# rushi-the-neural-arch/PyTorch-DistributedTraining

Measured on AMD Instinct MI355X. Metric: tokens/sec GPT-2-1.3B FSDP (whole node), higher is better.
Workload: dtype bf16; 1 GPU; model=gpt2-1.3b, global_batch=96, seq_len=1024, parallelism=fsdp1, micro_batch_per_gpu=96, params=1313722368, hip_graph=False, optimizer=fused AdamW + global-norm clip

## Files before the change

### csrc/kernels/gelu.h

```cpp
#pragma once
#include <hip/hip_runtime.h>

namespace pdt {

constexpr float kSqrt2OverPi = 0.7978845608028654f;
constexpr float kGeluC = 0.044715f;
constexpr float kInvSqrt2 = 0.7071067811865476f;

constexpr float kGeluA = -2.f * 0.7978845608028654f * 1.4426950408889634f;
constexpr float kGeluB = kGeluA * 0.044715f;
__device__ __forceinline__ float sigmoid2z(float u) {
  const float a = u * __builtin_fmaf(kGeluB, u * u, kGeluA);
  return __builtin_amdgcn_rcpf(1.f + __builtin_amdgcn_exp2f(a));
}

typedef float gelu_f32x2 __attribute__((ext_vector_type(2)));
constexpr float kGeluD1 = 2.f * 0.7978845608028654f;
constexpr float kGeluD3 = kGeluD1 * 3.f * 0.044715f;
__device__ __forceinline__ void gelu_fwd_grad2(gelu_f32x2 u, gelu_f32x2& y, gelu_f32x2& d) {
  const gelu_f32x2 u2 = u * u;
  const gelu_f32x2 a = u * __builtin_elementwise_fma(gelu_f32x2{kGeluB, kGeluB}, u2, gelu_f32x2{kGeluA, kGeluA});
  const gelu_f32x2 e = gelu_f32x2{__builtin_amdgcn_exp2f(a[0]), __builtin_amdgcn_exp2f(a[1])} + gelu_f32x2{1.f, 1.f};
  const gelu_f32x2 s = gelu_f32x2{__builtin_amdgcn_rcpf(e[0]), __builtin_amdgcn_rcpf(e[1])};
  y = u * s;
  const gelu_f32x2 t = __builtin_elementwise_fma(-s, s, s);
  const gelu_f32x2 q = __builtin_elementwise_fma(gelu_f32x2{kGeluD3, kGeluD3}, u2, gelu_f32x2{kGeluD1, kGeluD1});
  d = __builtin_elementwise_fma(u * t, q, s);
}

template <bool TANH>
__device__ __forceinline__ float gelu_f(float u) {
  if (TANH) {
    return u * sigmoid2z(u);
  } else {
    return 0.5f * u * (1.f + erff(u * kInvSqrt2));
  }
}
template <bool TANH>
__device__ __forceinline__ float gelu_grad(float u) {
  if (TANH) {
    const float s = sigmoid2z(u);
    return s + 2.f * u * s * (1.f - s) * kSqrt2OverPi * (1.f + 3.f * kGeluC * u * u);
  } else {
    const float cdf = 0.5f * (1.f + erff(u * kInvSqrt2));
    const float pdf = 0.3989422804014327f * __expf(-0.5f * u * u);
    return cdf + u * pdf;
  }
}

}
```

### csrc/kernels/gemm.hip

```cpp
#include "common.h"
#include "gelu.h"
#include "reduce.h"
#include <stdlib.h>
#include <type_traits>

using namespace pdt;

namespace {

typedef __bf16 bf16x8_t __attribute__((ext_vector_type(8)));
typedef short v4i16 __attribute__((ext_vector_type(4)));
typedef int v4i __attribute__((ext_vector_type(4)));
typedef __attribute__((address_space(3))) v4i16 lds_v4i16;
typedef __attribute__((address_space(3))) u16x8 lds_u16x8;
typedef __attribute__((address_space(3))) void lds_void;
typedef __attribute__((address_space(3))) const char lds_cchar;

constexpr int TM = 256, TN = 256, KB = 64, NTH = 256;
constexpr int OPB = TM * KB * 2;
constexpr int STB = 2 * OPB;
constexpr int PIECES = OPB / (NTH * 16);

enum { L_NT = 0, L_TT = 1 };
enum { E_PLAIN = 0, E_BIAS = 1, E_GELU = 2, E_DGELU = 3, E_F32 = 4 };

__device__ __forceinline__ f32x4 mfma16(const u16x8& a, const u16x8& b, const f32x4& c) {
  return __builtin_amdgcn_mfma_f32_16x16x32_bf16(__builtin_bit_cast(bf16x8_t, a), __builtin_bit_cast(bf16x8_t, b),
                                                 c, 0, 0, 0);
}

__device__ __forceinline__ int tt_f(int r) { return 2 * ((r & 3) | ((r >> 1) & 4)); }

template <int LAYOUT>
struct Dma {
  uint32_t off0, off1;
  uint32_t rowstep;
  __device__ __forceinline__ void init(int64_t ld, int w, int lane) {
    if (LAYOUT == L_NT) {
      const int row = 8 * w + (lane >> 3);
      const int c = (lane & 7) ^ ((row >> 1) & 7);
      off0 = off1 = (uint32_t)(row * ld * 2 + c * 16);
      rowstep = (uint32_t)(32 * ld * 2);
    } else {
      const int r0 = 2 * w + (lane >> 5);
      off0 = (uint32_t)(r0 * ld * 2 + ((lane & 31) ^ tt_f(r0)) * 16);
      off1 = (uint32_t)(r0 * ld * 2 + ((lane & 31) ^ tt_f(r0 + 8)) * 16);
      rowstep = (uint32_t)(8 * ld * 2);
    }
  }
  struct Tile {
    v4i rsrc;
    uint32_t lds0, rs;
  };
  __device__ __forceinline__ Tile tile(const char* t, uint32_t nbytes, uint32_t lds_op, int w) const {
    const uint64_t addr = (uint64_t)(uintptr_t)t;
    Tile d;
    d.rsrc[0] = __builtin_amdgcn_readfirstlane((int)(uint32_t)addr);
    d.rsrc[1] = __builtin_amdgcn_readfirstlane((int)((addr >> 32) & 0xffff));
    d.rsrc[2] = __builtin_amdgcn_readfirstlane((int)nbytes);
    d.rsrc[3] = 0x00020000;
    d.lds0 = __builtin_amdgcn_readfirstlane(lds_op + w * 1024);
    d.rs = __builtin_amdgcn_readfirstlane(rowstep);
    return d;
  }
  template <int I>
  __device__ __forceinline__ void piece(const Tile& d) const {
    asm volatile("s_mov_b32 m0, %0\n\tbuffer_load_dwordx4 %1, %2, %3 offen lds"
                 :: "s"(d.lds0 + I * 4096), "v"((I & 1) ? off1 : off0), "s"(d.rsrc), "s"(I * d.rs) : "memory");
  }
  template <int I0, int I1>
  __device__ __forceinline__ void issue(const char* tile, uint32_t nbytes, uint32_t lds_op, int w) const {
    const uint64_t addr = (uint64_t)(uintptr_t)tile;
    v4i rsrc;
    rsrc[0] = __builtin_amdgcn_readfirstlane((int)(uint32_t)addr);
    rsrc[1] = __builtin_amdgcn_readfirstlane((int)((addr >> 32) & 0xffff));
    rsrc[2] = __builtin_amdgcn_readfirstlane((int)nbytes);
    rsrc[3] = 0x00020000;
    const uint32_t lds0 = __builtin_amdgcn_readfirstlane(lds_op + w * 1024);
    const uint32_t rs = __builtin_amdgcn_readfirstlane(rowstep);
#pragma unroll
    for (int i = I0; i < I1; ++i) {
      const uint32_t m0 = lds0 + i * 4096;
      asm volatile("s_mov_b32 m0, %0\n\tbuffer_load_dwordx4 %1, %2, %3 offen lds"
                   :: "s"(m0), "v"((i & 1) ? off1 : off0), "s"(rsrc), "s"(i * rs) : "memory");
    }
  }
};

template <int LAYOUT>
struct Frag {
  uint32_t o0, o1;
  __device__ __forceinline__ void init(int lane) {
    const int x = lane & 15, g = lane >> 4;
    if (LAYOUT == L_NT) {
      const int h = (x >> 1) & 7;
      o0 = (uint32_t)(x * 128 + 16 * (g ^ h));
      o1 = (uint32_t)(x * 128 + 16 * ((4 + g) ^ h));
    } else {
      const int q = (lane >> 2) & 3, p = lane & 3;
      o0 = (uint32_t)((8 * g + q) * 512 + 16 * (p >> 1) + 8 * (p & 1));
      o1 = (uint32_t)tt_f(8 * g + q);
    }
  }
  template <int S>
  __device__ __forceinline__ u16x8 read(lds_cchar* op, int blk) const {
    if (LAYOUT == L_NT) {
      return *(const lds_u16x8*)(op + blk * 16 * 128 + (S ? o1 : o0));
    } else {
      const uint32_t a = o0 + S * 32 * 512 + 16 * ((uint32_t)(2 * blk) ^ o1);
      const v4i16 x = __builtin_amdgcn_ds_read_tr16_b64_v4i16((lds_v4i16*)(op + a));
      const v4i16 y = __builtin_amdgcn_ds_read_tr16_b64_v4i16((lds_v4i16*)(op + a + 2048));
      return __builtin_bit_cast(u16x8, __builtin_shufflevector(x, y, 0, 1, 2, 3, 4, 5, 6, 7));
    }
  }
};

struct GemmArgs {
  const bf16_t* A;
  const bf16_t* B;
  void* C;
  const bf16_t* bias;
  const bf16_t* aux;
  bf16_t* aux_out;
  float* ws;
  int M, N, K;
  int64_t lda, ldb, ldc;
  int k_per_split;
  int xpr;
  int grp;
};

__device__ __forceinline__ void tile_of(const GemmArgs& p, int id, int ntiles, int& tm, int& tn) {
  const int mt = p.M / TM, nt = p.N / TN;
  const int xcd = id & 7, loc = id >> 3;
  if (p.xpr > 0) {
    const int xpc = 8 / p.xpr, rb = mt / p.xpr, cb = nt / xpc, g = p.grp, per = g * cb;
    tm = (xcd / xpc) * rb + (loc / per) * g + loc % g;
    tn = (xcd % xpc) * cb + (loc % per) / g;
  } else {
    const int q8 = ntiles >> 3, r8 = ntiles & 7;
    const int t = (xcd < r8 ? xcd * (q8 + 1) : r8 * (q8 + 1) + (xcd - r8) * q8) + loc;
    tm = t / nt;
    tn = t % nt;
  }
}

template <int LAYOUT, int EPI>
__global__ __launch_bounds__(NTH, 1) void gemm_kernel(GemmArgs p) {
  __shared__ __attribute__((aligned(16))) char smem[2 * STB];
  lds_cchar* const lds = (lds_cchar*)(lds_void*)smem;
  const uint32_t lds_addr = (uint32_t)(uintptr_t)(lds_void*)smem;
  const int tid = threadIdx.x, w = tid >> 6, lane = tid & 63;
  const int wr = w >> 1, wc = w & 1;
  const int ntiles = (int)gridDim.x;
  int tm, tn;
  tile_of(p, blockIdx.x, ntiles, tm, tn);
  const int m0 = tm * TM, n0 = tn * TN;
  const int kbeg = blockIdx.y * p.k_per_split;
  const int T = min(p.K - kbeg, p.k_per_split) / KB;

  Dma<LAYOUT> da, db;
  da.init(p.lda, w, lane);
  db.init(p.ldb, w, lane);
  Frag<LAYOUT> fr;
  fr.init(lane);
  const char* Ab = reinterpret_cast<const char*>(p.A);
  const char* Bb = reinterpret_cast<const char*>(p.B);
  int64_t astep, bstep;
  uint32_t abytes, bbytes;
  auto tile_base = [&](int mm, int nn, int64_t& ao, int64_t& bo) {
    if (LAYOUT == L_NT) {
      ao = ((int64_t)mm * p.lda + kbeg) * 2; bo = ((int64_t)nn * p.ldb + kbeg) * 2;
    } else {
      ao = ((int64_t)kbeg * p.lda + mm) * 2; bo = ((int64_t)kbeg * p.ldb + nn) * 2;
    }
  };
  if (LAYOUT == L_NT) {
    astep = bstep = KB * 2;
    abytes = (uint32_t)((TM - 1) * p.lda * 2 + KB * 2); bbytes = (uint32_t)((TN - 1) * p.ldb * 2 + KB * 2);
  } else {
    astep = KB * p.lda * 2; bstep = KB * p.ldb * 2;
    abytes = (uint32_t)((KB - 1) * p.lda * 2 + TM * 2); bbytes = (uint32_t)((KB - 1) * p.ldb * 2 + TN * 2);
  }
  int64_t a0, b0;
  tile_base(m0, n0, a0, b0);
  auto issue = [&](auto i0, auto i1, int t) {
    constexpr int J0 = decltype(i0)::value, J1 = decltype(i1)::value;
    da.template issue<J0, J1>(Ab + a0 + t * astep, abytes, lds_addr + (t & 1) * STB, w);
    db.template issue<J0, J1>(Bb + b0 + t * bstep, bbytes, lds_addr + (t & 1) * STB + OPB, w);
  };
  using P0 = std::integral_constant<int, 0>;
  using PH = std::integral_constant<int, PIECES / 2>;
  using PE = std::integral_constant<int, PIECES>;

  f32x4 acc[8][8];
#pragma unroll
  for (int i = 0; i < 8; ++i)
#pragma unroll
    for (int j = 0; j < 8; ++j) acc[i][j] = f32x4{0.f, 0.f, 0.f, 0.f};
  u16x8 fa0[8], fb0[8], fa1[8], fb1[8];

  issue(P0{}, PE{}, 0);
  if (T > 1) issue(P0{}, PE{}, 1);
  if (T > 1) asm volatile("s_waitcnt vmcnt(%0)" :: "n"(2 * PIECES) : "memory");
  else asm volatile("s_waitcnt vmcnt(0)" ::: "memory");
  __builtin_amdgcn_s_barrier();
  asm volatile("" ::: "memory");
#pragma unroll
  for (int i = 0; i < 8; ++i) fa0[i] = fr.template read<0>(lds, 8 * wr + i);
#pragma unroll
  for (int j = 0; j < 8; ++j) fb0[j] = fr.template read<0>(lds + OPB, 8 * wc + j);

  auto kstep = [&](auto guarded, const int t) {
    constexpr bool G = decltype(guarded)::value;
    lds_cchar* sa = lds + (t & 1) * STB;
    lds_cchar* na = lds + ((t + 1) & 1) * STB;
    if (t >= 1 && (!G || t + 1 < T)) issue(PH{}, PE{}, t + 1);
#pragma unroll
    for (int j = 0; j < 8; ++j) fb1[j] = fr.template read<1>(sa + OPB, 8 * wc + j);
#pragma unroll
    for (int i = 0; i < 8; ++i) fa1[i] = fr.template read<1>(sa, 8 * wr + i);
#pragma unroll
    for (int i = 0; i < 8; ++i)
#pragma unroll
      for (int j = 0; j < 8; ++j) acc[i][j] = mfma16(fb0[j], fa0[i], acc[i][j]);
    if (!G) {
#pragma unroll
      for (int g = 0; g < 16; ++g) {
        __builtin_amdgcn_sched_group_barrier(0x100, 1, 0);
        __builtin_amdgcn_sched_group_barrier(0x008, 4, 0);
      }
    }
#pragma unroll
    for (int i = 0; i < 4; ++i)
#pragma unroll
      for (int j = 0; j < 8; ++j) acc[i][j] = mfma16(fb1[j], fa1[i], acc[i][j]);
    asm volatile("s_waitcnt vmcnt(0) lgkmcnt(0)" ::: "memory");
    __builtin_amdgcn_sched_barrier(0);
    __builtin_amdgcn_s_barrier();
    __builtin_amdgcn_sched_barrier(0);
    asm volatile("" ::: "memory");
    if (!G || t + 2 < T) issue(P0{}, PH{}, t + 2);
    const bool more = !G || t + 1 < T;
    if (more) {
#pragma unroll
      for (int j = 0; j < 8; ++j) fb0[j] = fr.template read<0>(na + OPB, 8 * wc + j);
#pragma unroll
      for (int i = 0; i < 8; ++i) fa0[i] = fr.template read<0>(na, 8 * wr + i);
    }
#pragma unroll
    for (int i = 4; i < 8; ++i)
#pragma unroll
      for (int j = 0; j < 8; ++j) acc[i][j] = mfma16(fb1[j], fa1[i], acc[i][j]);
    if (!G) {
#pragma unroll
      for (int g = 0; g < 16; ++g) {
        __builtin_amdgcn_sched_group_barrier(0x100, 1, 1);
        __builtin_amdgcn_sched_group_barrier(0x008, 2, 1);
      }
    }
  };
  using Steady = std::integral_constant<bool, false>;
  using Guarded = std::integral_constant<bool, true>;
  int t = 0;
  for (; t + 2 < T; ++t) kstep(Steady{}, t);
  for (; t < T; ++t) kstep(Guarded{}, t);

  {
  const int mrow = m0 + 128 * wr + (lane & 15);
  const int ncol = n0 + 128 * wc + 4 * (lane >> 4);
  if constexpr (EPI == E_F32) {
    float* C = p.ws + (int64_t)blockIdx.y * p.M * p.N;
#pragma unroll
    for (int i = 0; i < 8; ++i)
#pragma unroll
      for (int j = 0; j < 8; ++j)
        *reinterpret_cast<f32x4*>(C + (int64_t)(mrow + 16 * i) * p.N + ncol + 16 * j) = acc[i][j];
  } else {
    bf16_t* C = reinterpret_cast<bf16_t*>(p.C);
    float bj[8][4];
    if constexpr (EPI == E_BIAS || EPI == E_GELU) {
#pragma unroll
      for (int j = 0; j < 8; ++j) {
        const u16x4 b = *reinterpret_cast<const u16x4*>(p.bias + ncol + 16 * j);
#pragma unroll
        for (int r = 0; r < 4; ++r) bj[j][r] = bf2f(b[r]);
      }
    }
    float cs[8][4];
#pragma unroll
    for (int j = 0; j < 8; ++j)
#pragma unroll
      for (int r = 0; r < 4; ++r) cs[j][r] = 0.f;
#pragma unroll
    for (int i = 0; i < 8; ++i) {
      const int64_t rowoff = (int64_t)(mrow + 16 * i) * p.ldc;
#pragma unroll
      for (int j = 0; j < 8; ++j) {
        const int64_t e = rowoff + ncol + 16 * j;
        u16x4 o;
        if constexpr (EPI == E_PLAIN) {
#pragma unroll
          for (int r = 0; r < 4; ++r) o[r] = f2bf(acc[i][j][r]);
        } else if constexpr (EPI == E_BIAS) {
#pragma unroll
          for (int r = 0; r < 4; ++r) o[r] = f2bf(acc[i][j][r] + bj[j][r]);
        } else if constexpr (EPI == E_GELU) {
          u16x4 dd;
#pragma unroll
          for (int r = 0; r < 4; r += 2) {
            gelu_f32x2 y2, d2;
            gelu_fwd_grad2(gelu_f32x2{bf2f(f2bf(acc[i][j][r] + bj[j][r])), bf2f(f2bf(acc[i][j][r + 1] + bj[j][r + 1]))},
                           y2, d2);
            o[r] = f2bf(y2[0]); o[r + 1] = f2bf(y2[1]);
            dd[r] = f2bf(d2[0]); dd[r + 1] = f2bf(d2[1]);
          }
          *reinterpret_cast<u16x4*>(p.aux_out + e) = dd;
        } else {
          const u16x4 h = *reinterpret_cast<const u16x4*>(p.aux + e);
#pragma unroll
          for (int r = 0; r < 4; ++r) {
            const float g = acc[i][j][r] * bf2f(h[r]);
            const bf16_t gb = f2bf(g);
            o[r] = gb;
            cs[j][r] += bf2f(gb);
          }
        }
        *reinterpret_cast<u16x4*>(C + e) = o;
      }
    }
    if constexpr (EPI == E_DGELU) {
#pragma unroll
      for (int j = 0; j < 8; ++j)
#pragma unroll
        for (int r = 0; r < 4; ++r) {
          float v = cs[j][r];
          v += __shfl_xor(v, 1);
          v += __shfl_xor(v, 2);
          v += __shfl_xor(v, 4);
          v += __shfl_xor(v, 8);
          cs[j][r] = v;
        }
      __syncthreads();
      float* red = reinterpret_cast<float*>(smem);
      if ((lane & 15) == 0) {
#pragma unroll
        for (int j = 0; j < 8; ++j)
#pragma unroll
          for (int r = 0; r < 4; ++r) red[wr * 256 + 128 * wc + 16 * j + 4 * (lane >> 4) + r] = cs[j][r];
      }
      __syncthreads();
      p.ws[(int64_t)tm * p.N + n0 + tid] = red[tid] + red[256 + tid];
    }
  }
  }
}

}
#include "gemm_kloop.inc"
namespace {

constexpr int RING = 2 * STB;
constexpr int STAGE_BYTES = 32768;
constexpr int SMEM3 = RING + STAGE_BYTES;

template <int I, int N, class F>
__device__ __forceinline__ void sfor(F&& f) {
  if constexpr (I < N) {
    f(std::integral_constant<int, I>{});
    sfor<I + 1, N>(f);
  }
}

template <int K>
__device__ __forceinline__ f32x4 acc_tile() {
  float x, y, z, w;
  asm volatile("v_accvgpr_read_b32 %0, a%c4\n\tv_accvgpr_read_b32 %1, a%c5\n\t"
               "v_accvgpr_read_b32 %2, a%c6\n\tv_accvgpr_read_b32 %3, a%c7"
               : "=v"(x), "=v"(y), "=v"(z), "=v"(w)
               : "i"(4 * K), "i"(4 * K + 1), "i"(4 * K + 2), "i"(4 * K + 3));
  return f32x4{x, y, z, w};
}

__device__ __forceinline__ uint32_t stg_off(int q, int col) {
  return (uint32_t)(q * 512 + ((((col >> 3) ^ q) & 15) | ((col >> 3) & 16)) * 16 + (col & 7) * 2);
}
__device__ __forceinline__ int stg_row(int r, int q) { return 128 * (q >> 5) + 32 * r + (q & 31); }
__device__ __forceinline__ void stg_read(const char* img, u16x8 (&buf)[8], int w, int lane) {
#pragma unroll
  for (int it = 0; it < 8; ++it) {
    const int q = 16 * w + 2 * it + (lane >> 5), c16 = lane & 31;
    buf[it] = *reinterpret_cast<const u16x8*>(img + q * 512 + ((c16 ^ (q & 15)) & 15 | (c16 & 16)) * 16);
  }
}
typedef unsigned int u32x4 __attribute__((ext_vector_type(4)));
__device__ __forceinline__ __amdgpu_buffer_rsrc_t tile_rsrc(const bf16_t* base, int64_t ldc, int m0, int n0) {
  return __builtin_amdgcn_make_buffer_rsrc((void*)(base + (int64_t)m0 * ldc + n0), (short)0,
                                           (int)((255 * ldc + 256) * 2), 0x00020000);
}
__device__ __forceinline__ uint32_t stg_voff(int64_t ldc, int w, int lane) {
  return (uint32_t)(128 * (w >> 1) + 16 * (w & 1) + (lane >> 5)) * ((uint32_t)ldc * 2u) + (uint32_t)(lane & 31) * 16u;
}
__device__ __forceinline__ float row16_sum(float v) {
  v += __int_as_float(__builtin_amdgcn_update_dpp(0, __float_as_int(v), 0xB1, 0xF, 0xF, false));
  v += __int_as_float(__builtin_amdgcn_update_dpp(0, __float_as_int(v), 0x4E, 0xF, 0xF, false));
  v += __int_as_float(__builtin_amdgcn_update_dpp(0, __float_as_int(v), 0x141, 0xF, 0xF, false));
  v += __int_as_float(__builtin_amdgcn_update_dpp(0, __float_as_int(v), 0x140, 0xF, 0xF, false));
  return v;
}
__device__ __forceinline__ void stg_write_out(const u16x8 (&buf)[8], __amdgpu_buffer_rsrc_t rs, uint32_t vo,
                                              uint32_t ldc2, int r) {
#pragma unroll
  for (int it = 0; it < 8; ++it)
    __builtin_amdgcn_raw_buffer_store_b128(__builtin_bit_cast(u32x4, buf[it]), rs, (int)vo,
                                           (int)((32 * r + 2 * it) * ldc2), 0);
}
__device__ __forceinline__ void stg_fetch(u16x8 (&t)[8], __amdgpu_buffer_rsrc_t rs, uint32_t vo, uint32_t ldc2, int r) {
#pragma unroll
  for (int it = 0; it < 8; ++it)
    t[it] = __builtin_bit_cast(u16x8, __builtin_amdgcn_raw_buffer_load_b128(rs, (int)vo,
                                                                            (int)((32 * r + 2 * it) * ldc2), 0));
}
__device__ __forceinline__ void stg_put(char* img, const u16x8 (&t)[8], int w, int lane) {
#pragma unroll
  for (int it = 0; it < 8; ++it) {
    const int q = 16 * w + 2 * it + (lane >> 5), c16 = lane & 31;
    *reinterpret_cast<u16x8*>(img + q * 512 + ((c16 ^ (q & 15)) & 15 | (c16 & 16)) * 16) = t[it];
  }
}
__device__ __forceinline__ void stg_dma_round0(const bf16_t* src, int64_t ldc, int m0, int n0, uint32_t img_lds,
                                               int w, int lane) {
  const uint64_t base = (uint64_t)(uintptr_t)(src + (int64_t)m0 * ldc + n0);
  v4i rsrc;
  rsrc[0] = (int)(uint32_t)base;
  rsrc[1] = (int)((base >> 32) & 0xffff);
  rsrc[2] = (int)(uint32_t)((255 * ldc + 256) * 2);
  rsrc[3] = 0x00020000;
  const int hi = lane >> 5, p = lane & 31;
  const uint32_t row0 = (uint32_t)(128 * (w >> 1) + 16 * (w & 1));
  const uint32_t ldc2 = (uint32_t)ldc * 2u;
  uint32_t vo[8], so[8];
#pragma unroll
  for (int i = 0; i < 8; ++i) {
    const uint32_t c16 = (uint32_t)(((p ^ (2 * i + hi)) & 15) | (p & 16));
    vo[i] = (uint32_t)hi * ldc2 + c16 * 16u;
    so[i] = __builtin_amdgcn_readfirstlane((row0 + 2 * i) * ldc2);
  }
  const uint32_t m = __builtin_amdgcn_readfirstlane(img_lds + 16 * w * 512);
  asm volatile(
      "s_mov_b32 m0, %[m]\n\ts_nop 0\n\tbuffer_load_dwordx4 %[v0], %[rs], %[s0] offen lds\n\t"
      "s_add_u32 m0, m0, 1024\n\ts_nop 0\n\tbuffer_load_dwordx4 %[v1], %[rs], %[s1] offen lds\n\t"
      "s_add_u32 m0, m0, 1024\n\ts_nop 0\n\tbuffer_load_dwordx4 %[v2], %[rs], %[s2] offen lds\n\t"
      "s_add_u32 m0, m0, 1024\n\ts_nop 0\n\tbuffer_load_dwordx4 %[v3], %[rs], %[s3] offen lds\n\t"
      "s_add_u32 m0, m0, 1024\n\ts_nop 0\n\tbuffer_load_dwordx4 %[v4], %[rs], %[s4] offen lds\n\t"
      "s_add_u32 m0, m0, 1024\n\ts_nop 0\n\tbuffer_load_dwordx4 %[v5], %[rs], %[s5] offen lds\n\t"
      "s_add_u32 m0, m0, 1024\n\ts_nop 0\n\tbuffer_load_dwordx4 %[v6], %[rs], %[s6] offen lds\n\t"
      "s_add_u32 m0, m0, 1024\n\ts_nop 0\n\tbuffer_load_dwordx4 %[v7], %[rs], %[s7] offen lds"
      :
      : [m] "s"(m), [rs] "s"(rsrc), [v0] "v"(vo[0]), [v1] "v"(vo[1]), [v2] "v"(vo[2]), [v3] "v"(vo[3]),
        [v4] "v"(vo[4]), [v5] "v"(vo[5]), [v6] "v"(vo[6]), [v7] "v"(vo[7]), [s0] "s"(so[0]), [s1] "s"(so[1]),
        [s2] "s"(so[2]), [s3] "s"(so[3]), [s4] "s"(so[4]), [s5] "s"(so[5]), [s6] "s"(so[6]), [s7] "s"(so[7])
      : "memory", "scc");
}

__device__ __forceinline__ int item_tid(int wv) {
  int l;
  asm volatile("v_mbcnt_lo_u32_b32 %0, -1, 0\n\tv_mbcnt_hi_u32_b32 %0, -1, %0" : "=v"(l));
  return wv * 64 + l;
}
__device__ __forceinline__ int opaque_s(int x) {
  asm volatile("" : "+s"(x));
  return x;
}

__device__ __forceinline__ v4i scalar_rsrc(const void* base, uint32_t nbytes) {
  const uint64_t a = (uint64_t)(uintptr_t)base;
  v4i r;
  r[0] = (int)(uint32_t)a; r[1] = (int)((a >> 32) & 0xffff); r[2] = (int)nbytes; r[3] = 0x00020000;
  return r;
}
__device__ __forceinline__ void preload_bias(u16x4 (&b)[8], const bf16_t* bias, int n0, int lcol) {
  const v4i rs = scalar_rsrc(bias + n0, 512);
  const uint32_t vo = (uint32_t)lcol * 2u;
  asm volatile("buffer_load_dwordx2 %0, %8, %9, 0 offen offset:0\n\t"
               "buffer_load_dwordx2 %1, %8, %9, 0 offen offset:32\n\t"
               "buffer_load_dwordx2 %2, %8, %9, 0 offen offset:64\n\t"
               "buffer_load_dwordx2 %3, %8, %9, 0 offen offset:96\n\t"
               "buffer_load_dwordx2 %4, %8, %9, 0 offen offset:128\n\t"
               "buffer_load_dwordx2 %5, %8, %9, 0 offen offset:160\n\t"
               "buffer_load_dwordx2 %6, %8, %9, 0 offen offset:192\n\t"
               "buffer_load_dwordx2 %7, %8, %9, 0 offen offset:224"
               : "=&v"(b[0]), "=&v"(b[1]), "=&v"(b[2]), "=&v"(b[3]), "=&v"(b[4]), "=&v"(b[5]), "=&v"(b[6]),
                 "=&v"(b[7])
               : "v"(vo), "s"(rs)
               : "memory");
}
__device__ __forceinline__ void preload_round1(u16x8 (&t)[8], const bf16_t* src, int64_t ldc, int m0, int n0,
                                               uint32_t vo) {
  const v4i rs = scalar_rsrc(src + (int64_t)m0 * ldc + n0, (uint32_t)((255 * ldc + 256) * 2));
  const uint32_t l2 = (uint32_t)ldc * 2u;
  asm volatile("buffer_load_dwordx4 %0, %8, %9, %10 offen\n\t"
               "buffer_load_dwordx4 %1, %8, %9, %11 offen\n\t"
               "buffer_load_dwordx4 %2, %8, %9, %12 offen\n\t"
               "buffer_load_dwordx4 %3, %8, %9, %13 offen\n\t"
               "buffer_load_dwordx4 %4, %8, %9, %14 offen\n\t"
               "buffer_load_dwordx4 %5, %8, %9, %15 offen\n\t"
               "buffer_load_dwordx4 %6, %8, %9, %16 offen\n\t"
               "buffer_load_dwordx4 %7, %8, %9, %17 offen"
               : "=&v"(t[0]), "=&v"(t[1]), "=&v"(t[2]), "=&v"(t[3]), "=&v"(t[4]), "=&v"(t[5]), "=&v"(t[6]),
                 "=&v"(t[7])
               : "v"(vo), "s"(rs), "s"(32 * l2), "s"(34 * l2), "s"(36 * l2), "s"(38 * l2), "s"(40 * l2),
                 "s"(42 * l2), "s"(44 * l2), "s"(46 * l2)
               : "memory");
}
template <class V, int N>
__device__ __forceinline__ void settle(V (&x)[N]) {
#pragma unroll
  for (int i = 0; i < N; ++i) asm volatile("" : "+v"(x[i]));
}

template <int LAYOUT>
struct ItemOps {
  int tm, tn, m0, n0, split, T;
  uint32_t alo, ahi, blo, bhi;
  __device__ __forceinline__ void init(const GemmArgs& p, int item, int ntiles) {
    split = item / ntiles;
    tile_of(p, item - split * ntiles, ntiles, tm, tn);
    m0 = tm * TM; n0 = tn * TN;
    const int kbeg = split * p.k_per_split;
    T = min(p.K - kbeg, p.k_per_split) / KB;
    uint64_t a0, b0;
    if (LAYOUT == L_NT) {
      a0 = (uint64_t)(uintptr_t)p.A + ((uint64_t)m0 * p.lda + kbeg) * 2;
      b0 = (uint64_t)(uintptr_t)p.B + ((uint64_t)n0 * p.ldb + kbeg) * 2;
    } else {
      a0 = (uint64_t)(uintptr_t)p.A + ((uint64_t)kbeg * p.lda + m0) * 2;
      b0 = (uint64_t)(uintptr_t)p.B + ((uint64_t)kbeg * p.ldb + n0) * 2;
    }
    alo = (uint32_t)a0; ahi = (uint32_t)(a0 >> 32) & 0xffffu;
    blo = (uint32_t)b0; bhi = (uint32_t)(b0 >> 32) & 0xffffu;
  }
  __device__ __forceinline__ void skip2(uint64_t astep, uint64_t bstep) { skipn(2 * astep, 2 * bstep); }
  __device__ __forceinline__ void skip1(uint64_t astep, uint64_t bstep) { skipn(astep, bstep); }
  __device__ __forceinline__ void skipn(uint64_t da, uint64_t dbb) {
    const uint64_t a = (((uint64_t)ahi << 32) | alo) + da, b = (((uint64_t)bhi << 32) | blo) + dbb;
    alo = (uint32_t)a; ahi = (uint32_t)(a >> 32) & 0xffffu;
    blo = (uint32_t)b; bhi = (uint32_t)(b >> 32) & 0xffffu;
  }
};

__device__ __forceinline__ uint64_t stamp() {
  uint64_t t;
  asm volatile("s_memtime %0\n\ts_waitcnt lgkmcnt(0)" : "=s"(t) : : "memory");
  return t;
}

template <int LAYOUT, int EPI, int DIAG = 0, bool P3 = false>
__global__ __launch_bounds__(NTH, 1) void gemm_asm_kernel(GemmArgs p) {
  __shared__ __attribute__((aligned(16))) char smem[SMEM3];
  const uint32_t lds_addr = (uint32_t)(uintptr_t)(lds_void*)smem;
  const int tid = threadIdx.x, w = tid >> 6, lane = tid & 63;
  const int wr = w >> 1, wc = w & 1;
  const int wv = __builtin_amdgcn_readfirstlane(w);
  const int ntiles = (p.M / TM) * (p.N / TN);
  const int splits = (p.K + p.k_per_split - 1) / p.k_per_split;
  const int nall = ntiles * splits;

  uint64_t astep, bstep;
  uint32_t abytes, bbytes, rsa, rsb;
  int32_t db;
  if (LAYOUT == L_NT) {
    astep = bstep = KB * 2;
    abytes = (uint32_t)((TM - 1) * p.lda * 2 + KB * 2);
    bbytes = (uint32_t)((TN - 1) * p.ldb * 2 + KB * 2);
    rsa = (uint32_t)(32 * p.lda * 2);
    rsb = (uint32_t)(32 * p.ldb * 2);
    db = OPB + 16384 * (wc - wr);
  } else {
    astep = (uint64_t)KB * p.lda * 2;
    bstep = (uint64_t)KB * p.ldb * 2;
    abytes = (uint32_t)((KB - 1) * p.lda * 2 + TM * 2);
    bbytes = (uint32_t)((KB - 1) * p.ldb * 2 + TN * 2);
    rsa = (uint32_t)(8 * p.lda * 2);
    rsb = (uint32_t)(8 * p.ldb * 2);
    db = OPB + 256 * (wc - wr);
  }
  auto lane_ops = [&](int t, uint32_t& voa0, uint32_t& voa1, uint32_t& vob0, uint32_t& vob1, uint32_t& rd0,
                      uint32_t& rd1) {
    const int lw = t >> 6, ll = t & 63, lwr = lw >> 1;
    if (LAYOUT == L_NT) {
      const int row = 8 * lw + (ll >> 3);
      const int c = (ll & 7) ^ ((row >> 1) & 7);
      voa0 = voa1 = (uint32_t)(row * p.lda * 2 + c * 16);
      vob0 = vob1 = (uint32_t)(row * p.ldb * 2 + c * 16);
      const int x = ll & 15, g = ll >> 4, h = (x >> 1) & 7;
      rd0 = lds_addr + 16384 * lwr + (uint32_t)(x * 128 + 16 * (g ^ h));
      rd1 = lds_addr + 16384 * lwr + (uint32_t)(x * 128 + 16 * ((4 + g) ^ h));
    } else {
      const int r0 = 2 * lw + (ll >> 5);
      voa0 = (uint32_t)(r0 * p.lda * 2 + ((ll & 31) ^ tt_f(r0)) * 16);
      voa1 = (uint32_t)(r0 * p.lda * 2 + ((ll & 31) ^ tt_f(r0 + 8)) * 16);
      vob0 = (uint32_t)(r0 * p.ldb * 2 + ((ll & 31) ^ tt_f(r0)) * 16);
      vob1 = (uint32_t)(r0 * p.ldb * 2 + ((ll & 31) ^ tt_f(r0 + 8)) * 16);
      const int g = ll >> 4, q = (ll >> 2) & 3, pp = ll & 3;
      rd0 = lds_addr + 256 * lwr + (uint32_t)((8 * g + q) * 512 + 16 * (pp >> 1) + 8 * (pp & 1));
      rd1 = (uint32_t)tt_f(8 * g + q);
    }
  };
  const uint32_t m0b = __builtin_amdgcn_readfirstlane(lds_addr + w * 1024);
  const int dbs = __builtin_amdgcn_readfirstlane(db);
  const uint32_t asl = (uint32_t)astep, ash = (uint32_t)(astep >> 32);
  const uint32_t bsl = (uint32_t)bstep, bsh = (uint32_t)(bstep >> 32);
  constexpr int NST = EPI == E_F32 ? 64 : EPI == E_GELU ? 64 + 8 : EPI == E_DGELU ? 32 + 1 + 8 + 8 : EPI == E_BIAS ? 40 : 32;
  constexpr int WNX = 16 + NST < 63 ? 16 + NST : 63;
  char* const img = smem + RING;

#define PDT_KLOOP_CLOBBERS                                                                                      \
  "memory", "scc", "s80", "s81", "s82", "s83", "s84", "s85", "s86", "s87", "s88", "s89", "s90", "s91",         \
  "v64", "v65", "v66", "v67", "v68", "v69", "v70", "v71", "v72", "v73", "v74", "v75", "v76", "v77", "v78",     \
  "v79", "v80", "v81", "v82", "v83", "v84", "v85", "v86", "v87", "v88", "v89", "v90", "v91", "v92", "v93",     \
  "v94", "v95", "v128", "v129", "v130", "v131", "v132", "v133", "v134", "v135", "v136", "v137", "v138", "v139", \
  "v140", "v141", "v142", "v143", "v144", "v145", "v146", "v147", "v148", "v149", "v150", "v151", "v152",      \
  "v153", "v154", "v155", "v156", "v157", "v158", "v159", "v160", "v161", "v162", "v163", "v164", "v165",      \
  "v166", "v167", "v168", "v169", "v170", "v171", "v172", "v173", "v174", "v175", "v176", "v177", "v178",      \
  "v179", "v180", "v181", "v182", "v183", "v184", "v185", "v186", "v187", "v188", "v189", "v190", "v191",      \
  "v192", "v193", "v194", "v195", "v196", "v197", "v198", "v199", "v200", "v201", "v202", "v203", "v204",      \
  "v205", "v206", "v207", "v208", "v209", "v210", "v211", "v212", "v213", "v214", "v215", "v216", "v217",      \
  "v218", "v219", "v220", "v221", "v222", "v223", "v224", "v225", "v226", "v227", "v228", "v229", "v230",      \
  "v231", "v232", "v233", "v234", "v235", "v236", "v237", "v238", "v239", "v240", "v241", "v242", "v243",      \
  "v244", "v245", "v246", "v247", "v248", "v249", "v250", "v251", "v252", "v253", "v254", "v255",              \
  PDT_AGPR_CLOBBERS
#define PDT_ITEM_OPS                                                                                            \
  [alo] "s"(lo.alo), [ahi] "s"(lo.ahi), [anr] "s"(abytes), [blo] "s"(lo.blo), [bhi] "s"(lo.bhi),               \
      [bnr] "s"(bbytes), [m0b] "s"(m0b), [rsa] "s"(rsa), [rsb] "s"(rsb), [asl] "s"(asl), [ash] "s"(ash),         \
      [bsl] "s"(bsl), [bsh] "s"(bsh), [cnt] "s"(cnt), [first] "s"(first), [wnx] "i"(WNX), [hnx] "s"(hnx),        \
      [nalo] "s"(nxt.alo), [nahi] "s"(nxt.ahi), [nblo] "s"(nxt.blo), [nbhi] "s"(nxt.bhi), [db] "s"(dbs)
#define PDT_KLOOP_NT_ASM(MAC)                                                                                     \
  asm volatile(MAC : : PDT_ITEM_OPS, [voa] "v"(voa0), [vob] "v"(vob0), [rd0] "v"(rd0), [rd1] "v"(rd1)           \
               : PDT_KLOOP_CLOBBERS)
#define PDT_KLOOP_TT_ASM(MAC)                                                                                     \
  asm volatile(MAC : : PDT_ITEM_OPS, [voa0] "v"(voa0), [voa1] "v"(voa1), [vob0] "v"(vob0), [vob1] "v"(vob1),    \
               [rd0] "v"(rd0), [rdx] "v"(rd1) : PDT_KLOOP_CLOBBERS)
#define PDT_KLOOP_NT_ASM3(MAC)                                                                                    \
  asm volatile(MAC : : PDT_ITEM_OPS, [voa] "v"(voa0), [vob] "v"(vob0), [rd0] "v"(rd0), [rd1] "v"(rd1)           \
               : PDT_KLOOP_CLOBBERS, "v96", "v97")
#define PDT_KLOOP_TT_ASM3(MAC)                                                                                    \
  asm volatile(MAC : : PDT_ITEM_OPS, [voa0] "v"(voa0), [voa1] "v"(voa1), [vob0] "v"(vob0), [vob1] "v"(vob1),    \
               [rd0] "v"(rd0), [rdx] "v"(rd1)                                                                    \
               : PDT_KLOOP_CLOBBERS, "v96", "v97", "v98", "v99", "v100", "v101", "v102", "v103")
#define PDT_STAMP_OUTS                                                                                            \
  [st0] "=s"(ph[0]), [st1] "=s"(ph[1]), [st2] "=s"(ph[2]), [st3] "=s"(ph[3]), [st4] "=s"(ph[4]),               \
      [st5] "=s"(ph[5]), [st6] "=s"(ph[6]), [st7] "=s"(ph[7])
#define PDT_KLOOP_NT_ASM_ST(MAC)                                                                                  \
  asm volatile(MAC : PDT_STAMP_OUTS : PDT_ITEM_OPS, [voa] "v"(voa0), [vob] "v"(vob0), [rd0] "v"(rd0),            \
               [rd1] "v"(rd1) : PDT_KLOOP_CLOBBERS, "s92", "s93", "s94", "s95", "s96", "s97", "s98", "s99")
#define PDT_KLOOP_TT_ASM_ST(MAC)                                                                                  \
  asm volatile(MAC : PDT_STAMP_OUTS : PDT_ITEM_OPS, [voa0] "v"(voa0), [voa1] "v"(voa1), [vob0] "v"(vob0),         \
               [vob1] "v"(vob1), [rd0] "v"(rd0), [rdx] "v"(rd1)                                                  \
               : PDT_KLOOP_CLOBBERS, "s92", "s93", "s94", "s95", "s96", "s97", "s98", "s99")

  ItemOps<LAYOUT> cur;
  int item = blockIdx.x;
  cur.init(p, item, ntiles);
  int first = 1;
  while (true) {
    const int next_item = item + (int)gridDim.x;
    const bool has_next = next_item < nall;
    ItemOps<LAYOUT> nxt = cur;
    if (has_next) {
      GemmArgs q = p;
      q.M = opaque_s(p.M); q.N = opaque_s(p.N); q.xpr = opaque_s(p.xpr); q.grp = opaque_s(p.grp);
      q.K = opaque_s(p.K); q.k_per_split = opaque_s(p.k_per_split);
      nxt.init(q, next_item, opaque_s(ntiles));
    }
    const int hnx = P3 ? 0 : __builtin_amdgcn_readfirstlane((((nall - 1 - next_item) >> 31) + 1) & ~cur.T & 1);
    const int cnt = __builtin_amdgcn_readfirstlane(cur.T);
    first = __builtin_amdgcn_readfirstlane(first);
    ItemOps<LAYOUT> lo = cur;
    if (!first) lo.skip2(astep, bstep);
    lo.alo = __builtin_amdgcn_readfirstlane(lo.alo); lo.ahi = __builtin_amdgcn_readfirstlane(lo.ahi);
    lo.blo = __builtin_amdgcn_readfirstlane(lo.blo); lo.bhi = __builtin_amdgcn_readfirstlane(lo.bhi);
    uint64_t st0 = 0, st1 = 0, rt0 = 0;
    if (DIAG) { st0 = stamp(); rt0 = __builtin_amdgcn_s_memrealtime(); }
    const int ltid = item_tid(wv);
    uint32_t voa0, voa1, vob0, vob1, rd0, rd1;
    lane_ops(ltid, voa0, voa1, vob0, vob1, rd0, rd1);
    u16x4 pb[8];
    u16x8 pa[8];
    if constexpr (EPI == E_DGELU) {
      stg_dma_round0(p.aux, p.ldc, cur.m0, cur.n0, lds_addr + RING, ltid >> 6, ltid & 63);
      preload_round1(pa, p.aux, p.ldc, cur.m0, cur.n0, stg_voff(p.ldc, ltid >> 6, ltid & 63));
    }
    if constexpr (EPI == E_BIAS || EPI == E_GELU) preload_bias(pb, p.bias, cur.n0, 128 * ((ltid >> 6) & 1) + 4 * ((ltid & 63) >> 4));
    uint32_t ph[8] = {0, 0, 0, 0, 0, 0, 0, 0};
    if constexpr (DIAG) {
      if constexpr (LAYOUT == L_NT) PDT_KLOOP_NT_ASM_ST(PDT_GEMM_KLOOP_NT_STAMPS);
      else PDT_KLOOP_TT_ASM_ST(PDT_GEMM_KLOOP_TT_STAMPS);
    } else if constexpr (P3) {
      if constexpr (LAYOUT == L_NT) PDT_KLOOP_NT_ASM3(PDT_GEMM_KLOOP_NT3);
      else PDT_KLOOP_TT_ASM3(PDT_GEMM_KLOOP_TT3);
    } else {
      if constexpr (LAYOUT == L_NT) PDT_KLOOP_NT_ASM(PDT_GEMM_KLOOP_NT);
      else PDT_KLOOP_TT_ASM(PDT_GEMM_KLOOP_TT);
    }
    if constexpr (EPI == E_DGELU) settle(pa);
    if constexpr (EPI == E_BIAS || EPI == E_GELU) settle(pb);
    if (DIAG) st1 = stamp();
    const int m0 = cur.m0, n0 = cur.n0, tm = cur.tm;

    const int etid = item_tid(wv);
    {
    const int tid = etid, w = etid >> 6, lane = etid & 63, wr = w >> 1, wc = w & 1;
    const int lrow = 128 * wr + (lane & 15);
    const int lcol = 128 * wc + 4 * (lane >> 4);
    if constexpr (EPI == E_F32) {
      float* C = p.ws + (int64_t)cur.split * p.M * p.N;
      sfor<0, 64>([&](auto kc) {
        constexpr int k = decltype(kc)::value;
        const f32x4 v = acc_tile<k>();
        *reinterpret_cast<f32x4*>(C + (int64_t)(m0 + lrow + 16 * (k >> 3)) * p.N + n0 + lcol + 16 * (k & 7)) = v;
      });
    } else {
      bf16_t* C = reinterpret_cast<bf16_t*>(p.C);
      u16x8 buf[8];
      float bj[8][4];
      if constexpr (EPI == E_BIAS || EPI == E_GELU) {
#pragma unroll
        for (int j = 0; j < 8; ++j)
#pragma unroll
          for (int r = 0; r < 4; ++r) bj[j][r] = bf2f(pb[j][r]);
      }
      float cs[8][4];
#pragma unroll
      for (int j = 0; j < 8; ++j)
#pragma unroll
        for (int r = 0; r < 4; ++r) cs[j][r] = 0.f;
      u16x8 aux[2][8];
      const uint32_t svo = stg_voff(p.ldc, w, lane), ldc2 = (uint32_t)(p.ldc * 2);
      const __amdgpu_buffer_rsrc_t rsc = tile_rsrc(C, p.ldc, m0, n0);
      if constexpr (EPI == E_DGELU) {
#pragma unroll
        for (int it = 0; it < 8; ++it) aux[1][it] = pa[it];
      }
      sfor<0, 4>([&](auto rc) {
        constexpr int r = decltype(rc)::value;
        if constexpr (EPI == E_DGELU && r > 0) {
          __syncthreads();
          stg_put(img, aux[r & 1], w, lane);
          if constexpr (r < 3) stg_fetch(aux[(r + 1) & 1], tile_rsrc(p.aux, p.ldc, m0, n0), svo, ldc2, r + 1);
        }
        __syncthreads();
        u16x4 dk[16];
        u16x4 hk[8];
        sfor<0, 16>([&](auto kc) {
          constexpr int kk = decltype(kc)::value, k = 16 * r + kk, i = k >> 3, j = k & 7;
          if constexpr (EPI == E_DGELU && (kk & 7) == 0) {
            sfor<0, 8>([&](auto hc) {
              constexpr int k2 = k + decltype(hc)::value, i2 = k2 >> 3, j2 = k2 & 7;
              hk[decltype(hc)::value] = *reinterpret_cast<const u16x4*>(
                  img + stg_off(32 * wr + 16 * (i2 & 1) + (lane & 15), lcol + 16 * j2));
            });
          }
          const f32x4 v = acc_tile<k>();
          const uint32_t at = stg_off(32 * wr + 16 * (i & 1) + (lane & 15), lcol + 16 * j);
          u16x4 o;
          if constexpr (EPI == E_DGELU) {
            const u16x4 hh = hk[kk & 7];
#pragma unroll
            for (int e = 0; e < 4; ++e) {
              const bf16_t gb = f2bf(v[e] * bf2f(hh[e]));
              o[e] = gb;
              cs[j][e] += bf2f(gb);
            }
          } else if constexpr (EPI == E_GELU) {
#pragma unroll
            for (int e = 0; e < 4; e += 2) {
              gelu_f32x2 y2, d2;
              gelu_fwd_grad2(gelu_f32x2{bf2f(f2bf(v[e] + bj[j][e])), bf2f(f2bf(v[e + 1] + bj[j][e + 1]))}, y2, d2);
              o[e] = f2bf(y2[0]); o[e + 1] = f2bf(y2[1]);
              dk[kk][e] = f2bf(d2[0]); dk[kk][e + 1] = f2bf(d2[1]);
            }
          } else {
#pragma unroll
            for (int e = 0; e < 4; ++e) o[e] = f2bf(EPI == E_BIAS ? v[e] + bj[j][e] : v[e]);
          }
          *reinterpret_cast<u16x4*>(img + at) = o;
        });
        __syncthreads();
        stg_read(img, buf, w, lane);
        stg_write_out(buf, rsc, svo, ldc2, r);
        if constexpr (EPI == E_GELU) {
          __syncthreads();
          sfor<0, 16>([&](auto kc) {
            constexpr int kk = decltype(kc)::value, k = 16 * r + kk, i = k >> 3, j = k & 7;
            const uint32_t at = stg_off(32 * wr + 16 * (i & 1) + (lane & 15), lcol + 16 * j);
            *reinterpret_cast<u16x4*>(img + at) = dk[kk];
          });
          __syncthreads();
          stg_read(img, buf, w, lane);
          stg_write_out(buf, tile_rsrc(p.aux_out, p.ldc, m0, n0), svo, ldc2, r);
        }
      });
      if constexpr (EPI == E_DGELU) {
#pragma unroll
        for (int j = 0; j < 8; ++j)
#pragma unroll
          for (int e = 0; e < 4; ++e) cs[j][e] = row16_sum(cs[j][e]);
        __syncthreads();
        float* red = reinterpret_cast<float*>(img);
        if ((lane & 15) == 0) {
#pragma unroll
          for (int j = 0; j < 8; ++j)
#pragma unroll
            for (int e = 0; e < 4; ++e) red[wr * 256 + lcol + 16 * j + e] = cs[j][e];
        }
        __syncthreads();
        p.ws[(int64_t)tm * p.N + n0 + tid] = red[tid] + red[256 + tid];
      }
      __syncthreads();
    }
    }
    if (DIAG) {
      const uint64_t st2 = stamp();
      if (tid == 0) {
        uint64_t* d = reinterpret_cast<uint64_t*>(p.ws) + 8 * (int64_t)item;
        d[0] = st0; d[1] = st1; d[2] = st2; d[3] = rt0;
        for (int i = 0; i < 4; ++i) d[4 + i] = ((uint64_t)ph[2 * i + 1] << 32) | ph[2 * i];
      }
    }
    if (!has_next) break;
    item = next_item;
    first = 1 - hnx;
    cur = nxt;
  }
#undef PDT_KLOOP_CLOBBERS
#undef PDT_ITEM_OPS
#undef PDT_KLOOP_NT_ASM3
#undef PDT_KLOOP_TT_ASM3
#undef PDT_KLOOP_NT_ASM_ST
#undef PDT_KLOOP_TT_ASM_ST
#undef PDT_STAMP_OUTS
#undef PDT_KLOOP_NT_ASM
#undef PDT_KLOOP_TT_ASM
}

static int persist_grid(int nitems) {
  static const int cus = [] {
    int dev = 0, n = 0;
    if (hipGetDevice(&dev) != hipSuccess || hipDeviceGetAttribute(&n, hipDeviceAttributeMultiprocessorCount, dev) !=
                                                hipSuccess)
      n = 256;
    return n;
  }();
  int g = cus < nitems ? cus : nitems;
  return g >= 8 ? g & ~7 : g;
}

bool use_p3(int layout, const GemmArgs& a, int items, int grid) {
  static const int forced = [] { const char* e = getenv("PDT_GEMM_P3"); return e ? atoi(e) : -1; }();
  const int T = a.k_per_split / KB;
  if (T < 6 || forced == 0) return false;
  if (forced == 1) return true;
  const int cb = a.xpr > 0 ? (a.N / TN) / (8 / a.xpr) : a.N / TN;
  return layout == L_TT ? (items > grid && (a.M / TM) * (a.N / TN) < grid) : (a.k_per_split >= 8192 || cb <= 8);
}

template <int LAYOUT>
int launch_asm_layout(int epi, const GemmArgs& a, int splits, hipStream_t s) {
  const int items = (a.M / TM) * (a.N / TN) * splits;
  const dim3 grid(persist_grid(items), 1);
  if (use_p3(LAYOUT, a, items, (int)grid.x) && (epi == E_PLAIN || epi == E_BIAS || epi == E_F32)) {
    switch (epi) {
      case E_PLAIN: gemm_asm_kernel<LAYOUT, E_PLAIN, 0, true><<<grid, NTH, 0, s>>>(a); break;
      case E_BIAS: gemm_asm_kernel<LAYOUT, E_BIAS, 0, true><<<grid, NTH, 0, s>>>(a); break;
      default: gemm_asm_kernel<LAYOUT, E_F32, 0, true><<<grid, NTH, 0, s>>>(a); break;
    }
    return (int)hipGetLastError();
  }
  switch (epi) {
    case E_PLAIN: gemm_asm_kernel<LAYOUT, E_PLAIN><<<grid, NTH, 0, s>>>(a); break;
    case E_BIAS: gemm_asm_kernel<LAYOUT, E_BIAS><<<grid, NTH, 0, s>>>(a); break;
    case E_GELU: gemm_asm_kernel<LAYOUT, E_GELU><<<grid, NTH, 0, s>>>(a); break;
    case E_DGELU: gemm_asm_kernel<LAYOUT, E_DGELU><<<grid, NTH, 0, s>>>(a); break;
    case E_F32: gemm_asm_kernel<LAYOUT, E_F32><<<grid, NTH, 0, s>>>(a); break;
    default: return (int)hipErrorInvalidValue;
  }
  return (int)hipGetLastError();
}

__global__ __launch_bounds__(256) void gemm_splitk_reduce_kernel(const float* __restrict__ part,
                                                                 bf16_t* __restrict__ out, int64_t n4, int S,
                                                                 int64_t slab) {
  for (int64_t e = blockIdx.x * (int64_t)blockDim.x + threadIdx.x; e < n4; e += (int64_t)gridDim.x * blockDim.x) {
    f32x4 s = reinterpret_cast<const f32x4*>(part)[e];
    for (int k = 1; k < S; ++k) s += reinterpret_cast<const f32x4*>(part + k * slab)[e];
    u16x4 o;
#pragma unroll
    for (int r = 0; r < 4; ++r) o[r] = f2bf(s[r]);
    reinterpret_cast<u16x4*>(out)[e] = o;
  }
}


int xcd_grp(int mt, int nt, int K, int xpr) {
  if (xpr <= 0) return 1;
  const int rb = mt / xpr, cb = nt / (8 / xpr);
  static const int forced = [] { const char* e = getenv("PDT_GEMM_GRP"); return e ? atoi(e) : 0; }();
  if (forced > 0 && rb % forced == 0) return forced;
  const int pref[3] = {K <= 4096 ? 8 : 4, K <= 4096 ? 4 : 8, 2};
  for (int g : pref)
    if (rb % g == 0 && g * cb >= 16) return g;
  return 1;
}

int xcd_cut(int mt, int nt) {
  int xpr = 0, best = 1 << 30;
  for (int pr = 1; pr <= 8; pr *= 2) {
    const int pc = 8 / pr;
    if (mt % pr || nt % pc) continue;
    const int cost = mt / pr + nt / pc;
    if (cost < best) { best = cost; xpr = pr; }
  }
  return xpr;
}

template <int LAYOUT>
int launch_layout(int epi, const GemmArgs& a, int splits, hipStream_t s) {
  const dim3 grid((a.M / TM) * (a.N / TN), splits);
  switch (epi) {
    case E_PLAIN: gemm_kernel<LAYOUT, E_PLAIN><<<grid, NTH, 0, s>>>(a); break;
    case E_BIAS: gemm_kernel<LAYOUT, E_BIAS><<<grid, NTH, 0, s>>>(a); break;
    case E_GELU: gemm_kernel<LAYOUT, E_GELU><<<grid, NTH, 0, s>>>(a); break;
    case E_DGELU: gemm_kernel<LAYOUT, E_DGELU><<<grid, NTH, 0, s>>>(a); break;
    case E_F32: gemm_kernel<LAYOUT, E_F32><<<grid, NTH, 0, s>>>(a); break;
    default: return (int)hipErrorInvalidValue;
  }
  return (int)hipGetLastError();
}

}

PDT_API int pdt_gemm_ok(int layout, int64_t M, int64_t N, int64_t K, int64_t lda, int64_t ldb, int splits) {
  if (layout != L_NT && layout != L_TT) return 0;
  if (splits < 1 || M <= 0 || N <= 0 || K <= 0 || M % TM || N % TN || K % ((int64_t)KB * splits)) return 0;
  if ((M / TM) * (N / TN) > (1LL << 24) || lda % 8 || ldb % 8) return 0;
  if (layout == L_NT && (lda < K || ldb < K || (TM - 1) * lda * 2 + KB * 2 >= (1LL << 32) ||
                         (TN - 1) * ldb * 2 + KB * 2 >= (1LL << 32)))
    return 0;
  if (layout == L_TT && (lda < M || ldb < N || (KB - 1) * lda * 2 + TM * 2 >= (1LL << 32) ||
                         (KB - 1) * ldb * 2 + TN * 2 >= (1LL << 32)))
    return 0;
  return M <= (1LL << 30) && N <= (1LL << 30) && K <= (1LL << 30) ? 1 : 0;
}

PDT_API int pdt_gemm_bf16(int layout, int epi, const void* A, const void* B, void* C, int64_t M, int64_t N, int64_t K,
                          int64_t lda, int64_t ldb, int64_t ldc, const void* bias, const void* aux, void* aux_out,
                          void* dbias, float* ws, int splits, hipStream_t s) {
  if (!pdt_gemm_ok(layout, M, N, K, lda, ldb, splits) || ldc < N || ldc % 4) return (int)hipErrorInvalidValue;
  if (epi < 0 || epi > E_DGELU) return (int)hipErrorInvalidValue;
  if (splits > 1 && (epi != E_PLAIN || !ws)) return (int)hipErrorInvalidValue;
  if ((epi == E_BIAS || epi == E_GELU) && !bias) return (int)hipErrorInvalidValue;
  if (epi == E_GELU && !aux_out) return (int)hipErrorInvalidValue;
  if (epi == E_DGELU && (!aux || !ws || !dbias)) return (int)hipErrorInvalidValue;
  GemmArgs a{};
  a.A = (const bf16_t*)A; a.B = (const bf16_t*)B; a.C = C;
  a.bias = (const bf16_t*)bias; a.aux = (const bf16_t*)aux; a.aux_out = (bf16_t*)aux_out; a.ws = ws;
  a.M = (int)M; a.N = (int)N; a.K = (int)K; a.lda = lda; a.ldb = ldb; a.ldc = ldc;
  a.k_per_split = (int)(K / splits);
  a.xpr = xcd_cut((int)(M / TM), (int)(N / TN));
  a.grp = xcd_grp((int)(M / TM), (int)(N / TN), (int)(K / splits), a.xpr);
  const int run_epi = splits > 1 ? E_F32 : epi;
  if (splits > 1) a.ldc = N;
  int err = layout == L_NT ? launch_layout<L_NT>(run_epi, a, splits, s) : launch_layout<L_TT>(run_epi, a, splits, s);
  if (err) return err;
  if (splits > 1) {
    const int64_t n4 = M * N / 4;
    gemm_splitk_reduce_kernel<<<grid_for(n4, 256, 256 * 16), 256, 0, s>>>(ws, (bf16_t*)C, n4, splits, M * N);
    if (ldc != N) return (int)hipErrorInvalidValue;
  }
  if (epi == E_DGELU)
    red::col_reduce<bf16_t>(ws, (int)(M / TM), (int)N, (bf16_t*)dbias, ws + (M / TM) * N, 0, s);
  return (int)hipGetLastError();
}

PDT_API int pdt_gemm2_bf16(int layout, int epi, const void* A, const void* B, void* C, int64_t M, int64_t N,
                           int64_t K, int64_t lda, int64_t ldb, int64_t ldc, const void* bias, const void* aux,
                           void* aux_out, void* dbias, float* ws, int splits, hipStream_t s) {
  if (!pdt_gemm_ok(layout, M, N, K, lda, ldb, splits) || ldc < N || ldc % 8) return (int)hipErrorInvalidValue;
  if (K / splits < 2 * KB) return (int)hipErrorInvalidValue;
  if (epi < 0 || epi > E_DGELU) return (int)hipErrorInvalidValue;
  if (splits > 1 && (epi != E_PLAIN || !ws)) return (int)hipErrorInvalidValue;
  if ((epi == E_BIAS || epi == E_GELU) && !bias) return (int)hipErrorInvalidValue;
  if (epi == E_GELU && !aux_out) return (int)hipErrorInvalidValue;
  if (epi == E_DGELU && (!aux || !ws || !dbias)) return (int)hipErrorInvalidValue;
  GemmArgs a{};
  a.A = (const bf16_t*)A; a.B = (const bf16_t*)B; a.C = C;
  a.bias = (const bf16_t*)bias; a.aux = (const bf16_t*)aux; a.aux_out = (bf16_t*)aux_out; a.ws = ws;
  a.M = (int)M; a.N = (int)N; a.K = (int)K; a.lda = lda; a.ldb = ldb; a.ldc = ldc;
  a.k_per_split = (int)(K / splits);
  a.xpr = xcd_cut((int)(M / TM), (int)(N / TN));
  a.grp = xcd_grp((int)(M / TM), (int)(N / TN), (int)(K / splits), a.xpr);
  const int run_epi = splits > 1 ? E_F32 : epi;
  if (splits > 1) a.ldc = N;
  int err = layout == L_NT ? launch_asm_layout<L_NT>(run_epi, a, splits, s)
                           : launch_asm_layout<L_TT>(run_epi, a, splits, s);
  if (err) return err;
  if (splits > 1) {
    if (ldc != N) return (int)hipErrorInvalidValue;
    const int64_t n4 = M * N / 4;
    gemm_splitk_reduce_kernel<<<grid_for(n4, 256, 256 * 16), 256, 0, s>>>(ws, (bf16_t*)C, n4, splits, M * N);
  }
  if (epi == E_DGELU)
    red::col_reduce<bf16_t>(ws, (int)(M / TM), (int)N, (bf16_t*)dbias, ws + (M / TM) * N, 0, s);
  return (int)hipGetLastError();
}

PDT_API int pdt_gemm_stamps_epi_bf16(int layout, int epi, const void* A, const void* B, void* C, int64_t M, int64_t N,
                                     int64_t K, int64_t lda, int64_t ldb, const void* bias, void* aux_out,
                                     void* stamps, hipStream_t s);
PDT_API int pdt_gemm_stamps_bf16(int layout, const void* A, const void* B, void* C, int64_t M, int64_t N, int64_t K,
                                 int64_t lda, int64_t ldb, void* stamps, hipStream_t s) {
  if (!pdt_gemm_ok(layout, M, N, K, lda, ldb, 1) || K < 2 * KB || !stamps) return (int)hipErrorInvalidValue;
  return pdt_gemm_stamps_epi_bf16(layout, E_PLAIN, A, B, C, M, N, K, lda, ldb, nullptr, nullptr, stamps, s);
}

PDT_API int pdt_gemm_stamps_epi_bf16(int layout, int epi, const void* A, const void* B, void* C, int64_t M, int64_t N,
                                     int64_t K, int64_t lda, int64_t ldb, const void* bias, void* aux_out,
                                     void* stamps, hipStream_t s) {
  if (!pdt_gemm_ok(layout, M, N, K, lda, ldb, 1) || K < 2 * KB || !stamps) return (int)hipErrorInvalidValue;
  if (epi != E_PLAIN && (layout != L_NT || !bias || (epi == E_GELU && !aux_out) || (epi != E_BIAS && epi != E_GELU)))
    return (int)hipErrorInvalidValue;
  GemmArgs a{};
  a.A = (const bf16_t*)A; a.B = (const bf16_t*)B; a.C = C; a.ws = (float*)stamps;
  a.bias = (const bf16_t*)bias; a.aux_out = (bf16_t*)aux_out;
  a.M = (int)M; a.N = (int)N; a.K = (int)K; a.lda = lda; a.ldb = ldb; a.ldc = N; a.k_per_split = (int)K;
  a.xpr = xcd_cut((int)(M / TM), (int)(N / TN));
  a.grp = xcd_grp((int)(M / TM), (int)(N / TN), (int)K, a.xpr);
  const dim3 grid(persist_grid((int)((M / TM) * (N / TN))), 1);
  if (layout == L_TT) gemm_asm_kernel<L_TT, E_PLAIN, 1><<<grid, NTH, 0, s>>>(a);
  else if (epi == E_BIAS) gemm_asm_kernel<L_NT, E_BIAS, 1><<<grid, NTH, 0, s>>>(a);
  else if (epi == E_GELU) gemm_asm_kernel<L_NT, E_GELU, 1><<<grid, NTH, 0, s>>>(a);
  else gemm_asm_kernel<L_NT, E_PLAIN, 1><<<grid, NTH, 0, s>>>(a);
  return (int)hipGetLastError();
}
```

### pytorch_distributedtraining_amd/ops/gemm.py

```python
from __future__ import annotations

import os

import torch

from . import _lib

L_NT, L_TT = 0, 1
E_PLAIN, E_BIAS, E_GELU, E_DGELU = 0, 1, 2, 3


def gemm_ok(layout: int, m: int, n: int, k: int, lda: int, ldb: int, splits: int = 1) -> bool:
    return bool(_lib.require().pdt_gemm_ok(layout, m, n, k, lda, ldb, splits))


def _bf16_2d(t: torch.Tensor) -> bool:
    return t.is_cuda and t.dtype == torch.bfloat16 and t.dim() == 2 and t.stride(1) == 1 and t.data_ptr() % 16 == 0


def nt_ok(a: torch.Tensor, b: torch.Tensor) -> bool:
    return (_bf16_2d(a) and _bf16_2d(b) and a.shape[1] == b.shape[1]
            and gemm_ok(L_NT, a.shape[0], b.shape[0], a.shape[1], a.stride(0), b.stride(0)))


def tt_ok(a: torch.Tensor, b: torch.Tensor, splits: int = 1) -> bool:
    return (_bf16_2d(a) and _bf16_2d(b) and a.shape[0] == b.shape[0]
            and gemm_ok(L_TT, a.shape[1], b.shape[1], a.shape[0], a.stride(0), b.stride(0), splits))


KERNEL = {"name": os.environ.get("PDT_GEMM_KERNEL", "asm")}


def _launch(layout, epi, a, b, c, m, n, k, bias=None, aux=None, aux_out=None, dbias=None, ws=None, splits=1):
    asm = KERNEL["name"] == "asm" and k // splits >= 128 and c.stride(0) % 8 == 0
    fn = "pdt_gemm2_bf16" if asm else "pdt_gemm_bf16"
    _lib.call(fn, layout, epi, a.data_ptr(), b.data_ptr(), c.data_ptr(), m, n, k, a.stride(0),
              b.stride(0), c.stride(0), _lib.ptr(bias), _lib.ptr(aux), _lib.ptr(aux_out), _lib.ptr(dbias),
              _lib.ptr(ws), splits, _lib.stream_handle(a.device))


def gemm_nt(a: torch.Tensor, b: torch.Tensor, bias: torch.Tensor | None = None) -> torch.Tensor:
    m, k = a.shape
    n = b.shape[0]
    c = torch.empty(m, n, dtype=torch.bfloat16, device=a.device)
    _launch(L_NT, E_BIAS if bias is not None else E_PLAIN, a, b, c, m, n, k, bias=bias)
    return c


def gemm_nt_gelu(a: torch.Tensor, b: torch.Tensor, bias: torch.Tensor):
    m, k = a.shape
    n = b.shape[0]
    y = torch.empty(m, n, dtype=torch.bfloat16, device=a.device)
    d = torch.empty_like(y)
    _launch(L_NT, E_GELU, a, b, y, m, n, k, bias=bias, aux_out=d)
    return y, d


def gemm_nt_dgelu(a: torch.Tensor, b: torch.Tensor, d: torch.Tensor, bias_dtype=torch.bfloat16):
    m, k = a.shape
    n = b.shape[0]
    g = torch.empty(m, n, dtype=torch.bfloat16, device=a.device)
    db = torch.empty(n, dtype=torch.bfloat16, device=a.device)
    ws = torch.empty((m // 256 + 64) * n, dtype=torch.float32, device=a.device)
    _launch(L_NT, E_DGELU, a, b, g, m, n, k, aux=d, dbias=db, ws=ws)
    return g, db.to(bias_dtype)


def tt_splits(m: int, n: int, k: int, cus: int = 256) -> int:
    tiles = (m // 256) * (n // 256)
    if tiles == 0:
        return 1
    if tiles >= cus:
        eff1 = tiles / (-(-tiles // cus) * cus)
        best, best_eff = 1, eff1
        if eff1 < 0.9:
            for s in (2, 4):
                if k % (32 * s) or k // s < 4096:
                    break
                eff = s * tiles / (-(-(s * tiles) // cus) * cus)
                if eff > best_eff + 0.03:
                    best, best_eff = s, eff
        return best if best_eff > eff1 + 0.05 else 1
    best, best_eff = 1, 0.0
    for s in (1, 2, 4, 8, 16):
        if s > 1 and (k % (32 * s) or k // s < 4096):
            break
        wgs = tiles * s
        eff = wgs / (-(-wgs // cus) * cus)
        if eff > best_eff + 1e-9:
            best, best_eff = s, eff
    return best


def gemm_tt(a: torch.Tensor, b: torch.Tensor, splits: int | None = None, out: torch.Tensor | None = None) -> torch.Tensor:
    k, m = a.shape
    n = b.shape[1]
    s = splits or tt_splits(m, n, k)
    if out is not None:
        assert out.shape == (m, n) and out.dtype == torch.bfloat16 and out.is_contiguous()
    c = out if out is not None else torch.empty(m, n, dtype=torch.bfloat16, device=a.device)
    ws = torch.empty(s * m * n, dtype=torch.float32, device=a.device) if s > 1 else None
    _launch(L_TT, E_PLAIN, a, b, c, m, n, k, ws=ws, splits=s)
    return c
```

### pytorch_distributedtraining_amd/ops/linear.py

```python
from __future__ import annotations

import os

import torch
import torch.nn as nn
import torch.nn.functional as F

from . import _lib
from .activations import _colsum, colsum_ok
from .attention import stash_dx_colsum, take_bias_grad
from .blaslt import prefer_bgradb, wgrad_bgrad
from .fp8 import Fp8Meta, fp8_enabled, fp8_linear
from .gemm import gemm_tt, tt_ok, tt_splits
from .grad_slots import claim, is_sharded_param
from .narrow import narrow_linear, narrow_ok, narrow_wgrad, narrow_wgrad_ok
from .picks import timed_choice

_WGRAD_CHUNK = 4096
_DX_STASH = os.environ.get("PDT_DX_COLSUM_STASH", "1") == "1"


HIP_NT = os.environ.get("PDT_NT_HIP", "auto")
_NT_CHOICE: dict = {}


def _nt_hip_ok(a2: torch.Tensor, w: torch.Tensor, bias) -> bool:
    from . import gemm as G
    return (HIP_NT != "0" and G.KERNEL["name"] == "asm" and a2.is_cuda and a2.dim() == 2 and a2.shape[0] >= 4096
            and a2.dtype == torch.bfloat16 and w.dtype == torch.bfloat16 and w.is_contiguous()
            and (bias is None or (bias.dtype == torch.bfloat16 and bias.is_contiguous() and bias.data_ptr() % 16 == 0))
            and G.nt_ok(a2, w) and a2.shape[1] // 64 >= 2 and w.shape[0] % 8 == 0)


LT_NT = os.environ.get("PDT_NT_LT", "0")
_LT_CHOICE: dict = {}


def _lt_linear(a2, w, bias):
    from . import blaslt as LT
    m, k = a2.shape
    n = w.shape[0]
    y = torch.empty(m, n, dtype=a2.dtype, device=a2.device)
    if not LT.lt_matmul(LT.EPI_BIAS if bias is not None else LT.EPI_NONE, 1, n, m, k, w, a2, y, bias):
        return None
    return y


def _library_linear(a2, w, bias, key):
    if LT_NT != "0" and a2.is_cuda and a2.dtype == torch.bfloat16 and w.dtype == torch.bfloat16 \
            and a2.is_contiguous() and w.is_contiguous() and (bias is None or bias.dtype == torch.bfloat16):
        c = _LT_CHOICE.get(key)
        if c is None and not torch.cuda.is_current_stream_capturing():
            c = _LT_CHOICE[key] = _lt_linear(a2, w, bias) is not None and \
                timed_choice(lambda: _lt_linear(a2, w, bias), lambda: F.linear(a2, w, bias), 0.99,
                             table=_LT_CHOICE, key=key, name="lt")
        if c:
            y = _lt_linear(a2, w, bias)
            if y is not None:
                return y
    return F.linear(a2, w, bias)


def nt_matmul(a2: torch.Tensor, w: torch.Tensor, bias=None) -> torch.Tensor:
    key = (tuple(a2.shape), tuple(w.shape), bias is not None, a2.device)
    if _nt_hip_ok(a2, w, bias):
        from . import gemm as G
        if HIP_NT == "1":
            return G.gemm_nt(a2, w, bias)
        c = _NT_CHOICE.get(key)
        if c is None and not torch.cuda.is_current_stream_capturing():
            c = _NT_CHOICE[key] = timed_choice(lambda: G.gemm_nt(a2, w, bias),
                                               lambda: _library_linear(a2, w, bias, key), 0.99,
                                               table=_NT_CHOICE, key=key, name="nt")
        if c:
            return G.gemm_nt(a2, w, bias)
    return _library_linear(a2, w, bias, key)


NARROW = os.environ.get("PDT_NARROW", "auto")
_NARROW_CHOICE: dict = {}


def _prefer_narrow(x2: torch.Tensor, w: torch.Tensor, bias, role: str) -> bool:
    if NARROW == "0":
        return False
    if not narrow_ok(x2, w, bias, transposed=role != "fwd"):
        return False
    if NARROW == "1":
        return True
    key = (role, tuple(x2.shape), tuple(w.shape), bias is not None, x2.device)
    c = _NARROW_CHOICE.get(key)
    if c is None:
        if torch.cuda.is_current_stream_capturing():
            return True
        if role == "fwd":
            fa = lambda: narrow_linear(x2, w, bias)
            fb = lambda: F.linear(x2, w, bias)
        else:
            fa = lambda: narrow_linear(x2, w.t().contiguous(), None, w.dtype)
            fb = lambda: (torch.mm(x2, w), _colsum(x2, w.dtype) if colsum_ok(x2.shape[1]) else None)
        c = _NARROW_CHOICE[key] = timed_choice(fa, fb, table=_NARROW_CHOICE, key=key, name="narrow")
    return c


def _prefer_narrow_wgrad(dy2: torch.Tensor, x2: torch.Tensor, out_dtype: torch.dtype) -> bool:
    if NARROW == "0" or not narrow_wgrad_ok(dy2, x2, out_dtype):
        return False
    if NARROW == "1":
        return True
    key = ("wgrad", tuple(dy2.shape), x2.shape[1], out_dtype, dy2.device)
    c = _NARROW_CHOICE.get(key)
    if c is None:
        if torch.cuda.is_current_stream_capturing():
            return True
        c = _NARROW_CHOICE[key] = timed_choice(lambda: narrow_wgrad(dy2, x2, out_dtype),
                                               lambda: _library_wgrad(dy2, x2, out_dtype),
                                               table=_NARROW_CHOICE, key=key, name="narrow")
    return c


def _tall_skinny(m: int, n: int, k: int) -> bool:
    return m >= 16 * _WGRAD_CHUNK and max(n, k) <= 1024


def _split_k(m: int, n: int, k: int) -> int:
    nk = n * k
    if m < 8192 or nk > 2_500_000:
        return 1
    s = 8 if nk < 2_000_000 else 4
    while s > 1 and (m % s or m // s < 1024):
        s //= 2
    return s


HIP_WGRAD = os.environ.get("PDT_WGRAD_HIP", "auto")
_WGRAD_CHOICE: dict = {}


def _prefer_hip_wgrad(dy2: torch.Tensor, x2: torch.Tensor, ragged: bool = False) -> bool:
    if HIP_WGRAD != "auto":
        return HIP_WGRAD == "1"
    key = (dy2.shape, x2.shape[1], dy2.device)
    c = _WGRAD_CHOICE.get(key)
    if c is None:
        if torch.cuda.is_current_stream_capturing():
            return True
        hip = hip_wgrad_ragged if ragged else hip_wgrad
        c = _WGRAD_CHOICE[key] = timed_choice(lambda: hip(dy2, x2), lambda: _library_wgrad(dy2, x2, torch.bfloat16),
                                                    table=_WGRAD_CHOICE, key=key, name="wgrad")
    return c


def hip_wgrad_splits(m: int, n: int, k: int, cus: int = 256) -> int:
    return tt_splits(n, k, m, cus)


def hip_wgrad_ok(dy2: torch.Tensor, x2: torch.Tensor, out_dtype: torch.dtype) -> bool:
    m, n = dy2.shape
    k = x2.shape[1]
    return (HIP_WGRAD != "0" and dy2.is_cuda and out_dtype == torch.bfloat16 and m >= 4096
            and tt_ok(dy2, x2, hip_wgrad_splits(m, n, k)))


def hip_wgrad(dy2: torch.Tensor, x2: torch.Tensor, splits: int | None = None, out: torch.Tensor | None = None):
    m, n = dy2.shape
    k = x2.shape[1]
    return gemm_tt(dy2, x2, splits or hip_wgrad_splits(m, n, k), out=out)


def _ragged_rows(n: int) -> int:
    return n // 256 * 256


def hip_wgrad_ragged_ok(dy2: torch.Tensor, x2: torch.Tensor, out_dtype: torch.dtype) -> bool:
    m, n = dy2.shape
    k = x2.shape[1]
    nm = _ragged_rows(n)
    return (HIP_WGRAD != "0" and dy2.is_cuda and out_dtype == torch.bfloat16 and m >= 4096 and nm >= 4096
            and nm < n and tt_ok(dy2[:, :nm], x2, hip_wgrad_splits(m, nm, k)))


def hip_wgrad_ragged(dy2: torch.Tensor, x2: torch.Tensor, out: torch.Tensor | None = None) -> torch.Tensor:
    m, n = dy2.shape
    k = x2.shape[1]
    nm = _ragged_rows(n)
    if out is None:
        out = torch.empty(n, k, dtype=torch.bfloat16, device=dy2.device)
    gemm_tt(dy2[:, :nm], x2, hip_wgrad_splits(m, nm, k), out=out[:nm])
    if m % 16 == 0 and x2.is_contiguous():
        rest = dy2[:, nm:].contiguous()
        c = m // 16
        out[nm:].copy_(torch.bmm(rest.view(16, c, n - nm).transpose(1, 2), x2.view(16, c, k),
                                 out_dtype=torch.float32).sum(0))
    else:
        torch.mm(dy2[:, nm:].t(), x2, out=out[nm:])
    return out


def wgrad(dy2: torch.Tensor, x2: torch.Tensor, out_dtype: torch.dtype, out: torch.Tensor | None = None):
    m, n = dy2.shape
    k = x2.shape[1]
    if not dy2.is_cuda:
        r = torch.mm(dy2.t(), x2).to(out_dtype)
    elif hip_wgrad_ok(dy2, x2, out_dtype) and _prefer_hip_wgrad(dy2, x2):
        r = hip_wgrad(dy2, x2, out=out)
    elif hip_wgrad_ragged_ok(dy2, x2, out_dtype) and _prefer_hip_wgrad(dy2, x2, ragged=True):
        r = hip_wgrad_ragged(dy2, x2, out=out)
    elif _prefer_narrow_wgrad(dy2, x2, out_dtype):
        r = narrow_wgrad(dy2, x2, out_dtype)
    else:
        r = _library_wgrad(dy2, x2, out_dtype, out=out)
    if out is not None and r.data_ptr() != out.data_ptr():
        out.copy_(r)
        r = out
    return r


def _wgrad_result(w: torch.Tensor, dy2: torch.Tensor, x2: torch.Tensor):
    slot = claim(w)
    if slot is None:
        return wgrad(dy2, x2, w.dtype)
    dst, acc = slot
    if acc:
        dst.add_(wgrad(dy2, x2, w.dtype))
    else:
        wgrad(dy2, x2, w.dtype, out=dst)
    return None


def _library_wgrad(dy2: torch.Tensor, x2: torch.Tensor, out_dtype: torch.dtype, out: torch.Tensor | None = None):
    m, n = dy2.shape
    k = x2.shape[1]
    if not _tall_skinny(m, n, k):
        sk = _split_k(m, n, k)
        if sk == 1:
            if out is not None and out.dtype == dy2.dtype == x2.dtype:
                return torch.mm(dy2.t(), x2, out=out)
            return torch.mm(dy2.t(), x2).to(out_dtype)
        c = m // sk
        g = torch.bmm(dy2.view(sk, c, n).transpose(1, 2), x2.view(sk, c, k), out_dtype=torch.float32).sum(0)
        return g.to(out_dtype)
    s = m // _WGRAD_CHUNK
    main = s * _WGRAD_CHUNK
    a = dy2[:main].view(s, _WGRAD_CHUNK, n).transpose(1, 2)
    b = x2[:main].view(s, _WGRAD_CHUNK, k)
    g = torch.bmm(a, b, out_dtype=torch.float32).sum(0)
    if main < m:
        g += torch.mm(dy2[main:].t(), x2[main:], out_dtype=torch.float32)
    return g.to(out_dtype)


def transpose16(w: torch.Tensor) -> torch.Tensor:
    r, c = w.shape
    out = torch.empty(c, r, dtype=w.dtype, device=w.device)
    _lib.call("pdt_transpose16", w.data_ptr(), out.data_ptr(), r, c, _lib.stream_handle(w.device))
    return out


def _dgrad_via_transpose(m: int, n: int, k: int, w: torch.Tensor) -> bool:
    return (w.is_cuda and w.dtype in (torch.bfloat16, torch.float16) and w.is_contiguous() and m >= 4096
            and n % 64 == 0 and k % 64 == 0 and n * k >= _DGRAD_T_MIN and n // 64 <= 65535 and w.data_ptr() % 16 == 0)


_DGRAD_T_MIN = int(os.environ.get("PDT_DGRAD_T_MIN", "500000"))


BGRAD_IN_GEMM = os.environ.get("PDT_BGRAD_GEMM", "0") == "1"


def _bgrad_in_gemm(dy2: torch.Tensor, w: torch.Tensor) -> bool:
    m, n = dy2.shape
    k = w.shape[1]
    return (BGRAD_IN_GEMM and dy2.is_cuda and dy2.dtype == torch.bfloat16 and w.dtype == torch.bfloat16
            and not _tall_skinny(m, n, k) and _split_k(m, n, k) == 1 and n % 8 == 0 and k % 8 == 0 and colsum_ok(n))


def _as_output(t: torch.Tensor, shape) -> torch.Tensor:
    return torch.ops.aten._unsafe_view(t, shape)


class _LinearFn(torch.autograd.Function):
    @staticmethod
    def forward(ctx, x, weight, bias, hm=None, in_hm=None):
        ctx.save_for_backward(x, weight)
        ctx.in_hm = in_hm
        ctx.has_bias = bias is not None
        base = x._base if x._base is not None else x
        ctx.dx_colsum = bias is not None and getattr(base, "_pdt_dx_colsum", False)
        x2 = x.reshape(-1, x.shape[-1])
        if hm is not None:
            return _as_output(narrow_linear(x2, weight, bias, hm=hm)[0], (*x.shape[:-1], weight.shape[0]))
        if in_hm is not None:
            return _as_output(narrow_linear(x2, weight, bias, a_hm=in_hm)[0], (*x.shape[:-1], weight.shape[0]))
        if x2.is_contiguous() and _prefer_narrow(x2, weight, bias, "fwd"):
            return _as_output(narrow_linear(x2, weight, bias)[0], (*x.shape[:-1], weight.shape[0]))
        if x2.is_contiguous() and _nt_hip_ok(x2, weight, bias):
            return _as_output(nt_matmul(x2, weight, bias), (*x.shape[:-1], weight.shape[0]))
        return F.linear(x, weight, bias)

    @staticmethod
    def backward(ctx, dy):
        x, w = ctx.saved_tensors
        dy2 = dy.reshape(-1, dy.shape[-1])
        if not dy2.is_contiguous():
            dy2 = dy2.contiguous()
        if ctx.in_hm is not None:
            return _LinearFn._backward_head_major(ctx, x, w, dy, dy2) + (None, None)
        dx = dw = db = None
        want_db = ctx.has_bias and ctx.needs_input_grad[2]
        if ctx.needs_input_grad[1] and want_db and _bgrad_in_gemm(dy2, w):
            x2 = x.reshape(-1, x.shape[-1])
            x2 = x2 if x2.is_contiguous() else x2.contiguous()
            if prefer_bgradb(dy2, x2, lambda: (wgrad(dy2, x2, w.dtype), _colsum(dy2, w.dtype))):
                r = wgrad_bgrad(dy2, x2)
                if r is not None:
                    dw, db = r
                    want_db = False
        if ctx.needs_input_grad[1] and dw is None:
            x2 = x.reshape(-1, x.shape[-1])
            if not x2.is_contiguous():
                x2 = x2.contiguous()
            dw = _wgrad_result(w, dy2, x2)
        dx2 = dbf = None
        if ctx.needs_input_grad[0] and _prefer_narrow(dy2, w, None, "dgrad"):
            pre = take_bias_grad(dy2) if want_db else None
            dx2, cs = narrow_linear(dy2, w.t().contiguous(), None, w.dtype if (want_db and pre is None) else None)
            dx = dx2.view(*dy.shape[:-1], w.shape[1])
            if want_db:
                if pre is not None:
                    dbf, db = pre, pre.to(w.dtype)
                else:
                    db = cs
                want_db = False
        elif ctx.needs_input_grad[0]:
            if _dgrad_via_transpose(dy2.shape[0], w.shape[0], w.shape[1], w):
                dx2 = nt_matmul(dy2, transpose16(w))
            else:
                dx2 = torch.mm(dy2, w)
            dx = dx2.view(*dy.shape[:-1], w.shape[1])
        if want_db:
            db = take_bias_grad(dy2)
            if db is not None:
                dbf, db = db, db.to(w.dtype)
            else:
                db = _colsum(dy2, w.dtype) if (dy2.is_cuda and colsum_ok(dy2.shape[1])) else dy2.sum(0).to(w.dtype)
        if ctx.dx_colsum and _DX_STASH and dx is not None and db is not None:
            dbf = dbf if dbf is not None and dbf.dtype == torch.float32 else db.float()
            stash_dx_colsum(dx2, dbf @ w.float())
        return dx, dw, db, None, None

    @staticmethod
    def _backward_head_major(ctx, x, w, dy, dy2):
        n_tok, d = ctx.in_hm
        x2 = x.reshape(-1, x.shape[-1])
        dx = dw = db = None
        want_db = ctx.has_bias and ctx.needs_input_grad[2]
        if ctx.needs_input_grad[1]:
            if narrow_wgrad_ok(dy2, x2, w.dtype) and n_tok == 64:
                dw = narrow_wgrad(dy2, x2, w.dtype, x_hm_d=d)
            else:
                dw = wgrad(dy2, _token_major(x2, n_tok, d), w.dtype)
        if ctx.needs_input_grad[0]:
            wt = w.t().contiguous()
            if narrow_ok(dy2, wt):
                dx2, cs = narrow_linear(dy2, wt, None, w.dtype if want_db else None, hm=(n_tok, d))
                dx = dx2.view(*dy.shape[:-1], w.shape[1])
                dx._pdt_head_major = (n_tok, d)
                if want_db:
                    db, want_db = cs, False
            else:
                dx = torch.mm(dy2, w).view(*dy.shape[:-1], w.shape[1])
        if want_db:
            db = _colsum(dy2, w.dtype) if (dy2.is_cuda and colsum_ok(dy2.shape[1])) else dy2.sum(0).to(w.dtype)
        return dx, dw, db


def _token_major(x2: torch.Tensor, n_tok: int, d: int) -> torch.Tensor:
    M, C = x2.shape
    return x2.reshape(M // n_tok, C // d, n_tok, d).permute(0, 2, 1, 3).reshape(M, C)


def _lin_residual_fwd(x2, w, b, r2):
    from .blaslt import linear_residual as _lt_residual
    if x2.is_cuda and x2.dtype == torch.bfloat16 and w.dtype == torch.bfloat16 and r2.dtype == torch.bfloat16 \
            and (b is None or b.dtype == torch.bfloat16) and w.is_contiguous() and r2.is_contiguous():
        d = _lt_residual(x2, w, b, r2)
        if d is not None:
            return d
    return torch.addmm(r2, x2, w.t()) if b is None else F.linear(x2, w, b) + r2


class _LinearResidualFn(torch.autograd.Function):

    @staticmethod
    def forward(ctx, x, weight, bias, r):
        ctx.save_for_backward(x, weight)
        ctx.has_bias = bias is not None
        base = x._base if x._base is not None else x
        ctx.dx_colsum = bias is not None and getattr(base, "_pdt_dx_colsum", False)
        n = weight.shape[0]
        x2 = x.reshape(-1, x.shape[-1])
        x2 = x2 if x2.is_contiguous() else x2.contiguous()
        r2 = r.reshape(-1, n)
        r2 = r2 if r2.is_contiguous() else r2.contiguous()
        if r2.data_ptr() % 16 == 0 and r2.dtype == x2.dtype and _prefer_narrow(x2, weight, bias, "fwd"):
            return _as_output(narrow_linear(x2, weight, bias, residual=r2)[0], (*x.shape[:-1], n))
        return _as_output(_lin_residual_fwd(x2, weight, bias, r2), (*x.shape[:-1], n))

    @staticmethod
    def backward(ctx, dy):
        x, w = ctx.saved_tensors
        dy2 = dy.reshape(-1, dy.shape[-1])
        dy2 = dy2 if dy2.is_contiguous() else dy2.contiguous()
        dx = dx2 = dw = db = None
        if ctx.needs_input_grad[1]:
            x2 = x.reshape(-1, x.shape[-1])
            x2 = x2 if x2.is_contiguous() else x2.contiguous()
            dw = _wgrad_result(w, dy2, x2)
        dbf = None
        if ctx.needs_input_grad[0]:
            if _prefer_narrow(dy2, w, None, "dgrad"):
                want = ctx.has_bias and (ctx.needs_input_grad[2] or ctx.dx_colsum)
                pre = take_bias_grad(dy2) if want else None
                dx2, cs = narrow_linear(dy2, w.t().contiguous(), None, torch.float32 if (want and pre is None) else None)
                dbf = pre if pre is not None else cs
            elif _dgrad_via_transpose(dy2.shape[0], w.shape[0], w.shape[1], w):
                dx2 = nt_matmul(dy2, transpose16(w))
            else:
                dx2 = torch.mm(dy2, w)
            dx = dx2.view(*dy.shape[:-1], w.shape[1])
        if ctx.has_bias and (ctx.needs_input_grad[2] or ctx.dx_colsum):
            if dbf is None:
                dbf = take_bias_grad(dy2)
            if dbf is None:
                dbf = _colsum(dy2, torch.float32) if (dy2.is_cuda and colsum_ok(dy2.shape[1])) else dy2.float().sum(0)
            db = dbf.to(w.dtype)
            if ctx.dx_colsum and _DX_STASH and dx2 is not None:
                stash_dx_colsum(dx2, dbf.float() @ w.float())
            if not ctx.needs_input_grad[2]:
                db = None
        return dx, dw, db, (dy if ctx.needs_input_grad[3] else None)


def linear_residual(x, weight, bias, r):
    if x.is_cuda and x.dtype == weight.dtype == r.dtype and x.dtype in (torch.bfloat16, torch.float32) \
            and (bias is None or bias.dtype == x.dtype) and not torch.is_autocast_enabled("cuda"):
        return _LinearResidualFn.apply(x, weight, bias, r)
    return linear(x, weight, bias) + r


FUSED_GELU = os.environ.get("PDT_FUSED_GELU", "1") == "1"


def linear_bias_gelu_ok(x, weight, bias) -> bool:
    from . import gemm as G
    if not (FUSED_GELU and G.KERNEL["name"] == "asm" and x.is_cuda and bias is not None):
        return False
    if torch.is_autocast_enabled("cuda") or x.dtype != torch.bfloat16 or weight.dtype != torch.bfloat16 \
            or bias.dtype != torch.bfloat16 or not weight.is_contiguous():
        return False
    m = x.numel() // x.shape[-1]
    n, k = weight.shape
    return (m % 256 == 0 and n % 256 == 0 and k % 64 == 0 and k >= 128 and x.shape[-1] == k
            and G.gemm_ok(G.L_NT, m, n, k, k, k) and weight.data_ptr() % 16 == 0)


class _LinearBiasGeluFn(torch.autograd.Function):

    @staticmethod
    def forward(ctx, x, weight, bias):
        from . import gemm as G
        x2 = x.reshape(-1, x.shape[-1])
        x2 = x2 if x2.is_contiguous() and x2.data_ptr() % 16 == 0 else x2.contiguous()
        y, d = G.gemm_nt_gelu(x2, weight, bias)
        ctx.save_for_backward(x2, weight, d)
        ctx.xshape = x.shape
        return _as_output(y, (*x.shape[:-1], weight.shape[0]))

    @staticmethod
    def backward(ctx, dy):
        x2, w, d = ctx.saved_tensors
        dy2 = dy.reshape(d.shape)
        dy2 = dy2 if dy2.is_contiguous() else dy2.contiguous()
        rows, n = d.shape
        lib = _lib.require()
        dpre = torch.empty_like(d)
        db = torch.empty(n, dtype=w.dtype, device=d.device)
        ws = torch.empty(lib.pdt_colsum_ws_floats(rows, n), dtype=torch.float32, device=d.device)
        _lib.call("pdt_bias_gelu_bwd_db", dy2.data_ptr(), d.data_ptr(), None, dpre.data_ptr(),
                  db.data_ptr(), ws.data_ptr(), rows, n, _lib.dtype_code(d.dtype), _lib.dtype_code(db.dtype), 2, 0,
                  _lib.stream_handle(d.device))
        dw = _wgrad_result(w, dpre, x2) if ctx.needs_input_grad[1] else None
        dx = None
        if ctx.needs_input_grad[0]:
            if _dgrad_via_transpose(rows, w.shape[0], w.shape[1], w):
                dx = nt_matmul(dpre, transpose16(w))
            else:
                dx = torch.mm(dpre, w)
            dx = dx.view(*ctx.xshape)
        return dx, dw, (db if ctx.needs_input_grad[2] else None)


def linear_bias_gelu(x, weight, bias):
    return _LinearBiasGeluFn.apply(x, weight, bias)


FUSED_DGELU = os.environ.get("PDT_FUSED_DGELU", "1") == "1"


def gelu_mlp_ok(x, w1, b1, w2, b2) -> bool:
    return (FUSED_DGELU and linear_bias_gelu_ok(x, w1, b1) and w2.dtype == torch.bfloat16 and w2.is_contiguous()
            and b2 is not None and b2.dtype == torch.bfloat16 and w2.shape[1] == w1.shape[0]
            and w2.shape[0] % 64 == 0 and w2.shape[0] >= 128)


class _GeluMlpFn(torch.autograd.Function):

    @staticmethod
    def forward(ctx, x, w1, b1, w2, b2, r=None):
        from . import gemm as G
        x2 = x.reshape(-1, x.shape[-1])
        x2 = x2 if x2.is_contiguous() and x2.data_ptr() % 16 == 0 else x2.contiguous()
        y1, d1 = G.gemm_nt_gelu(x2, w1, b1)
        if r is None:
            out = F.linear(y1, w2, b2)
        else:
            r2 = r.reshape(-1, w2.shape[0])
            out = _lin_residual_fwd(y1, w2, b2, r2 if r2.is_contiguous() else r2.contiguous())
        ctx.save_for_backward(x2, w1, d1, y1, w2)
        ctx.xshape = x.shape
        ctx.has_r = r is not None
        return _as_output(out, (*x.shape[:-1], w2.shape[0]))

    @staticmethod
    def backward(ctx, dout):
        from . import gemm as G
        x2, w1, d1, y1, w2 = ctx.saved_tensors
        d2 = dout.reshape(-1, dout.shape[-1])
        d2 = d2 if d2.is_contiguous() and d2.data_ptr() % 16 == 0 else d2.contiguous()
        dw2 = _wgrad_result(w2, d2, y1) if ctx.needs_input_grad[3] else None
        db2 = None
        if ctx.needs_input_grad[4]:
            db2 = take_bias_grad(d2)
            db2 = db2.to(w2.dtype) if db2 is not None else _colsum(d2, w2.dtype)
        dpre, db1 = G.gemm_nt_dgelu(d2, transpose16(w2), d1, bias_dtype=w1.dtype)
        dw1 = _wgrad_result(w1, dpre, x2) if ctx.needs_input_grad[1] else None
        dx = None
        if ctx.needs_input_grad[0]:
            if _dgrad_via_transpose(dpre.shape[0], w1.shape[0], w1.shape[1], w1):
                dx = nt_matmul(dpre, transpose16(w1))
            else:
                dx = torch.mm(dpre, w1)
            dx = dx.view(*ctx.xshape)
        dr = dout if ctx.has_r and ctx.needs_input_grad[5] else None
        return dx, dw1, (db1 if ctx.needs_input_grad[2] else None), dw2, db2, dr


def gelu_mlp(x, w1, b1, w2, b2, residual=None):
    return _GeluMlpFn.apply(x, w1, b1, w2, b2, residual)


def linear(x, weight, bias=None):
    if x.is_cuda and torch.is_autocast_enabled("cuda"):
        dt = torch.get_autocast_dtype("cuda")
        with torch.autocast("cuda", enabled=False):
            return linear(x.to(dt), weight.to(dt), None if bias is None else bias.to(dt))
    if (x.is_cuda or is_sharded_param(weight) or hasattr(x, "_pdt_recipe")) and x.dtype == weight.dtype and \
            x.dtype in (torch.bfloat16, torch.float32) and (bias is None or bias.dtype == x.dtype):
        return _LinearFn.apply(x, weight, bias)
    return F.linear(x, weight, bias)


HEAD_MAJOR_QKV = os.environ.get("PDT_HEAD_MAJOR_QKV", "1") == "1"


def _has_hooks(module: nn.Module) -> bool:
    return bool(module._forward_hooks or module._forward_pre_hooks or nn.modules.module._global_forward_hooks
                or nn.modules.module._global_forward_pre_hooks)


def linear_head_major(module: "Linear", x: torch.Tensor, n_tok: int, head_dim: int) -> torch.Tensor:
    from .narrow import head_major_ok
    if HEAD_MAJOR_QKV and x.is_cuda and not fp8_enabled() and not _has_hooks(module):
        xc = x.to(torch.get_autocast_dtype("cuda")) if torch.is_autocast_enabled("cuda") else x
        w, b = module.weight, module.bias
        if torch.is_autocast_enabled("cuda"):
            w, b = w.to(xc.dtype), (None if b is None else b.to(xc.dtype))
        x2 = xc.reshape(-1, xc.shape[-1])
        if (xc.dtype == w.dtype and xc.dtype in (torch.bfloat16, torch.float32) and (b is None or b.dtype == xc.dtype)
                and x2.is_contiguous() and head_major_ok(x2.shape[0], w.shape[0], (n_tok, head_dim))
                and _prefer_narrow(x2, w, b, "fwd")):
            with torch.autocast("cuda", enabled=False):
                y = _LinearFn.apply(xc, w, b, (n_tok, head_dim))
            y._pdt_head_major = (n_tok, head_dim)
            return y
    return module(x)


def from_head_major_ok(module: "Linear", rows: int, dtype: torch.dtype) -> bool:
    if _has_hooks(module) or fp8_enabled() or dtype != torch.bfloat16:
        return False
    w, b = module.weight, module.bias
    if not torch.is_autocast_enabled("cuda") and (w.dtype != dtype or (b is not None and b.dtype != dtype)):
        return False
    if not (w.is_cuda and w.dim() == 2 and w.is_contiguous() and (b is None or b.is_contiguous())
            and rows >= 16384 and _lib.available()):
        return False
    return bool(_lib.require().pdt_narrow_gemm_ok(rows, w.shape[1], w.shape[0]))


class _TokenMajorFn(torch.autograd.Function):

    @staticmethod
    def forward(ctx, x, n_tok, d):
        ctx.hm = (n_tok, d)
        return _as_output(_token_major(x.reshape(-1, x.shape[-1]), n_tok, d).contiguous(), x.shape)

    @staticmethod
    def backward(ctx, g):
        n_tok, d = ctx.hm
        M, C = g.numel() // g.shape[-1], g.shape[-1]
        dx = g.reshape(M // n_tok, n_tok, C // d, d).permute(0, 2, 1, 3).contiguous().view(g.shape)
        dx._pdt_head_major = ctx.hm
        return dx, None, None


def linear_from_head_major(module: "Linear", x: torch.Tensor) -> torch.Tensor:
    hm = getattr(x, "_pdt_head_major", None)
    if hm is None:
        return module(x)
    n_tok, d = hm
    x2 = x.reshape(-1, x.shape[-1])
    if from_head_major_ok(module, x2.shape[0], x.dtype):
        w, b = module.weight, module.bias
        if torch.is_autocast_enabled("cuda"):
            w, b = w.to(x.dtype), (None if b is None else b.to(x.dtype))
        if x2.is_contiguous() and narrow_ok(x2, w, b):
            with torch.autocast("cuda", enabled=False):
                return _LinearFn.apply(x, w, b, None, hm)
    return module(_TokenMajorFn.apply(x, n_tok, d))


class Linear(nn.Linear):

    def _fp8_meta(self, x):
        if not (fp8_enabled() and x.dtype in (torch.bfloat16, torch.float16) and self.in_features % 16 == 0
                and self.out_features % 16 == 0):
            return None
        meta = self.__dict__.get("_fp8")
        if meta is None:
            meta = self.__dict__["_fp8"] = Fp8Meta(x.device)
        return meta

    def forward(self, x):
        return self.matmul(x, self.bias)

    def matmul(self, x, bias=None):
        if x.is_cuda and torch.is_autocast_enabled("cuda"):
            x = x.to(torch.get_autocast_dtype("cuda"))
        meta = self._fp8_meta(x)
        if meta is not None and x.shape[:-1].numel() % 16 == 0:
            w = self.weight if self.weight.dtype == x.dtype else self.weight.to(x.dtype)
            b = None if bias is None else bias.to(x.dtype)
            return fp8_linear(x, w, b, meta)
        return linear(x, self.weight, bias)
```

Measured before the change: 151,200 tokens/s.

## Store GELU derivative aux in per-tile fragment layout for fused MLP GEMMs

The GELU-forward GEMM now writes its saved derivative tensor in a tile-blocked, per-lane fragment order instead of row-major. The dgelu backward GEMM reads it back with direct 16-byte vector loads that match its accumulator layout, replacing the row-major staging through LDS and the extra syncs. This cuts epilogue shared-memory traffic and barriers in both MLP GEMMs. The cost is that the aux tensor is no longer usable as a normal row-major matrix, and register pressure rises from the preloaded fragments.

```diff
diff --git a/csrc/kernels/gelu.h b/csrc/kernels/gelu.h
--- a/csrc/kernels/gelu.h
+++ b/csrc/kernels/gelu.h
@@ -28,6 +28,30 @@
   d = __builtin_elementwise_fma(u * t, q, s);
 }
 
+template <int N>
+__device__ __forceinline__ void gelu_fwd_grad2n(const gelu_f32x2 (&u)[N], gelu_f32x2 (&y)[N], gelu_f32x2 (&d)[N]) {
+  gelu_f32x2 u2[N], a[N], e[N], s[N], t[N], q[N];
+#pragma unroll
+  for (int i = 0; i < N; ++i) u2[i] = u[i] * u[i];
+#pragma unroll
+  for (int i = 0; i < N; ++i)
+    a[i] = u[i] * __builtin_elementwise_fma(gelu_f32x2{kGeluB, kGeluB}, u2[i], gelu_f32x2{kGeluA, kGeluA});
+#pragma unroll
+  for (int i = 0; i < N; ++i)
+    e[i] = gelu_f32x2{__builtin_amdgcn_exp2f(a[i][0]), __builtin_amdgcn_exp2f(a[i][1])} + gelu_f32x2{1.f, 1.f};
+#pragma unroll
+  for (int i = 0; i < N; ++i) s[i] = gelu_f32x2{__builtin_amdgcn_rcpf(e[i][0]), __builtin_amdgcn_rcpf(e[i][1])};
+#pragma unroll
+  for (int i = 0; i < N; ++i) y[i] = u[i] * s[i];
+#pragma unroll
+  for (int i = 0; i < N; ++i) t[i] = __builtin_elementwise_fma(-s[i], s[i], s[i]);
+#pragma unroll
+  for (int i = 0; i < N; ++i)
+    q[i] = __builtin_elementwise_fma(gelu_f32x2{kGeluD3, kGeluD3}, u2[i], gelu_f32x2{kGeluD1, kGeluD1});
+#pragma unroll
+  for (int i = 0; i < N; ++i) d[i] = __builtin_elementwise_fma(u[i] * t[i], q[i], s[i]);
+}
+
 template <bool TANH>
 __device__ __forceinline__ float gelu_f(float u) {
   if (TANH) {
diff --git a/csrc/kernels/gemm.hip b/csrc/kernels/gemm.hip
--- a/csrc/kernels/gemm.hip
+++ b/csrc/kernels/gemm.hip
@@ -123,12 +123,21 @@
   const bf16_t* aux;
   bf16_t* aux_out;
   float* ws;
+  uint64_t* stamps;
   int M, N, K;
   int64_t lda, ldb, ldc;
   int k_per_split;
   int xpr;
   int grp;
 };
+
+constexpr int AUX_BLOCK = TM * TN;
+__device__ __forceinline__ uint32_t aux_frag_voff(int w, int lane) {
+  return (uint32_t)(w * 32768 + lane * 16);
+}
+__device__ __forceinline__ int64_t aux_frag_block(const GemmArgs& p, int tm, int tn) {
+  return ((int64_t)tm * (p.N / TN) + tn) * AUX_BLOCK;
+}
 
 __device__ __forceinline__ void tile_of(const GemmArgs& p, int id, int ntiles, int& tm, int& tn) {
   const int mt = p.M / TM, nt = p.N / TN;
@@ -145,7 +154,7 @@
   }
 }
 
-template <int LAYOUT, int EPI>
+template <int LAYOUT, int EPI, bool AUXF = false>
 __global__ __launch_bounds__(NTH, 1) void gemm_kernel(GemmArgs p) {
   __shared__ __attribute__((aligned(16))) char smem[2 * STB];
   lds_cchar* const lds = (lds_cchar*)(lds_void*)smem;
@@ -292,6 +301,9 @@
     for (int j = 0; j < 8; ++j)
 #pragma unroll
       for (int r = 0; r < 4; ++r) cs[j][r] = 0.f;
+    const int64_t fragoff = AUXF ? aux_frag_block(p, tm, tn) + aux_frag_voff(w, lane) / 2 : 0;
+    u16x4 dlo;
+    u16x8 hp;
 #pragma unroll
     for (int i = 0; i < 8; ++i) {
       const int64_t rowoff = (int64_t)(mrow + 16 * i) * p.ldc;
@@ -315,9 +327,22 @@
             o[r] = f2bf(y2[0]); o[r + 1] = f2bf(y2[1]);
             dd[r] = f2bf(d2[0]); dd[r + 1] = f2bf(d2[1]);
           }
-          *reinterpret_cast<u16x4*>(p.aux_out + e) = dd;
+          if constexpr (!AUXF) {
+            *reinterpret_cast<u16x4*>(p.aux_out + e) = dd;
+          } else if (j & 1) {
+            *reinterpret_cast<u16x8*>(p.aux_out + fragoff + 512 * ((8 * i + j) >> 1)) =
+                __builtin_shufflevector(dlo, dd, 0, 1, 2, 3, 4, 5, 6, 7);
+          } else {
+            dlo = dd;
+          }
         } else {
-          const u16x4 h = *reinterpret_cast<const u16x4*>(p.aux + e);
+          u16x4 h;
+          if constexpr (!AUXF) {
+            h = *reinterpret_cast<const u16x4*>(p.aux + e);
+          } else {
+            if (!(j & 1)) hp = *reinterpret_cast<const u16x8*>(p.aux + fragoff + 512 * ((8 * i + j) >> 1));
+            h = (j & 1) ? __builtin_shufflevector(hp, hp, 4, 5, 6, 7) : __builtin_shufflevector(hp, hp, 0, 1, 2, 3);
+          }
 #pragma unroll
           for (int r = 0; r < 4; ++r) {
             const float g = acc[i][j][r] * bf2f(h[r]);
@@ -513,6 +538,30 @@
                  "s"(42 * l2), "s"(44 * l2), "s"(46 * l2)
                : "memory");
 }
+__device__ __forceinline__ void preload_frag01(u16x8 (&t)[16], const bf16_t* blk, uint32_t vo) {
+  const v4i rs = scalar_rsrc(blk, (uint32_t)(AUX_BLOCK * 2));
+  asm volatile("buffer_load_dwordx4 %0, %16, %17, 0 offen\n\t"
+               "buffer_load_dwordx4 %1, %16, %17, 0 offen offset:1024\n\t"
+               "buffer_load_dwordx4 %2, %16, %17, 0 offen offset:2048\n\t"
+               "buffer_load_dwordx4 %3, %16, %17, 0 offen offset:3072\n\t"
+               "buffer_load_dwordx4 %4, %16, %17, %18 offen\n\t"
+               "buffer_load_dwordx4 %5, %16, %17, %18 offen offset:1024\n\t"
+               "buffer_load_dwordx4 %6, %16, %17, %18 offen offset:2048\n\t"
+               "buffer_load_dwordx4 %7, %16, %17, %18 offen offset:3072\n\t"
+               "buffer_load_dwordx4 %8, %16, %17, %19 offen\n\t"
+               "buffer_load_dwordx4 %9, %16, %17, %19 offen offset:1024\n\t"
+               "buffer_load_dwordx4 %10, %16, %17, %19 offen offset:2048\n\t"
+               "buffer_load_dwordx4 %11, %16, %17, %19 offen offset:3072\n\t"
+               "buffer_load_dwordx4 %12, %16, %17, %20 offen\n\t"
+               "buffer_load_dwordx4 %13, %16, %17, %20 offen offset:1024\n\t"
+               "buffer_load_dwordx4 %14, %16, %17, %20 offen offset:2048\n\t"
+               "buffer_load_dwordx4 %15, %16, %17, %20 offen offset:3072"
+               : "=&v"(t[0]), "=&v"(t[1]), "=&v"(t[2]), "=&v"(t[3]), "=&v"(t[4]), "=&v"(t[5]), "=&v"(t[6]),
+                 "=&v"(t[7]), "=&v"(t[8]), "=&v"(t[9]), "=&v"(t[10]), "=&v"(t[11]), "=&v"(t[12]), "=&v"(t[13]),
+                 "=&v"(t[14]), "=&v"(t[15])
+               : "v"(vo), "s"(rs), "s"(4096), "s"(8192), "s"(12288)
+               : "memory");
+}
 template <class V, int N>
 __device__ __forceinline__ void settle(V (&x)[N]) {
 #pragma unroll
@@ -555,7 +604,7 @@
   return t;
 }
 
-template <int LAYOUT, int EPI, int DIAG = 0, bool P3 = false>
+template <int LAYOUT, int EPI, int DIAG = 0, bool P3 = false, bool AUXF = false>
 __global__ __launch_bounds__(NTH, 1) void gemm_asm_kernel(GemmArgs p) {
   __shared__ __attribute__((aligned(16))) char smem[SMEM3];
   const uint32_t lds_addr = (uint32_t)(uintptr_t)(lds_void*)smem;
@@ -611,7 +660,8 @@
   const int dbs = __builtin_amdgcn_readfirstlane(db);
   const uint32_t asl = (uint32_t)astep, ash = (uint32_t)(astep >> 32);
   const uint32_t bsl = (uint32_t)bstep, bsh = (uint32_t)(bstep >> 32);
-  constexpr int NST = EPI == E_F32 ? 64 : EPI == E_GELU ? 64 + 8 : EPI == E_DGELU ? 32 + 1 + 8 + 8 : EPI == E_BIAS ? 40 : 32;
+  constexpr int NST_DGELU = AUXF ? 32 + 1 + 16 : 32 + 1 + 8 + 8;
+  constexpr int NST = EPI == E_F32 ? 64 : EPI == E_GELU ? 64 + 8 : EPI == E_DGELU ? NST_DGELU : EPI == E_BIAS ? 40 : 32;
   constexpr int WNX = 16 + NST < 63 ? 16 + NST : 63;
   char* const img = smem + RING;
 
@@ -687,12 +737,16 @@
     lane_ops(ltid, voa0, voa1, vob0, vob1, rd0, rd1);
     u16x4 pb[8];
     u16x8 pa[8];
-    if constexpr (EPI == E_DGELU) {
+    u16x8 pf[16];
+    if constexpr (EPI == E_DGELU && AUXF) {
+      preload_frag01(pf, p.aux + aux_frag_block(p, cur.tm, cur.tn), aux_frag_voff(ltid >> 6, ltid & 63));
+    } else if constexpr (EPI == E_DGELU) {
       stg_dma_round0(p.aux, p.ldc, cur.m0, cur.n0, lds_addr + RING, ltid >> 6, ltid & 63);
       preload_round1(pa, p.aux, p.ldc, cur.m0, cur.n0, stg_voff(p.ldc, ltid >> 6, ltid & 63));
     }
     if constexpr (EPI == E_BIAS || EPI == E_GELU) preload_bias(pb, p.bias, cur.n0, 128 * ((ltid >> 6) & 1) + 4 * ((ltid & 63) >> 4));
     uint32_t ph[8] = {0, 0, 0, 0, 0, 0, 0, 0};
+    if constexpr (EPI == E_DGELU && AUXF && !DIAG) asm volatile("s_nop 0");
     if constexpr (DIAG) {
       if constexpr (LAYOUT == L_NT) PDT_KLOOP_NT_ASM_ST(PDT_GEMM_KLOOP_NT_STAMPS);
       else PDT_KLOOP_TT_ASM_ST(PDT_GEMM_KLOOP_TT_STAMPS);
@@ -703,7 +757,8 @@
       if constexpr (LAYOUT == L_NT) PDT_KLOOP_NT_ASM(PDT_GEMM_KLOOP_NT);
       else PDT_KLOOP_TT_ASM(PDT_GEMM_KLOOP_TT);
     }
-    if constexpr (EPI == E_DGELU) settle(pa);
+    if constexpr (EPI == E_DGELU && AUXF) settle(pf);
+    else if constexpr (EPI == E_DGELU) settle(pa);
     if constexpr (EPI == E_BIAS || EPI == E_GELU) settle(pb);
     if (DIAG) st1 = stamp();
     const int m0 = cur.m0, n0 = cur.n0, tm = cur.tm;
@@ -738,13 +793,27 @@
       u16x8 aux[2][8];
       const uint32_t svo = stg_voff(p.ldc, w, lane), ldc2 = (uint32_t)(p.ldc * 2);
       const __amdgpu_buffer_rsrc_t rsc = tile_rsrc(C, p.ldc, m0, n0);
-      if constexpr (EPI == E_DGELU) {
+      if constexpr (EPI == E_DGELU && !AUXF) {
 #pragma unroll
         for (int it = 0; it < 8; ++it) aux[1][it] = pa[it];
+      }
+      u16x8 fa[2][8];
+      const uint32_t fvo = aux_frag_voff(w, lane);
+      __amdgpu_buffer_rsrc_t rsf;
+      if constexpr (AUXF && (EPI == E_GELU || EPI == E_DGELU))
+        rsf = __builtin_amdgcn_make_buffer_rsrc(
+            (void*)((EPI == E_GELU ? p.aux_out : const_cast<bf16_t*>(p.aux)) + aux_frag_block(p, tm, cur.tn)), (short)0,
+            AUX_BLOCK * 2, 0x00020000);
+      if constexpr (EPI == E_DGELU && AUXF) {
+        sfor<0, 16>([&](auto c) {
+          constexpr int kp = 16 + decltype(c)::value;
+          fa[(kp >> 3) & 1][kp & 7] =
+              __builtin_bit_cast(u16x8, __builtin_amdgcn_raw_buffer_load_b128(rsf, (int)fvo, 1024 * kp, 0));
+        });
       }
       sfor<0, 4>([&](auto rc) {
         constexpr int r = decltype(rc)::value;
-        if constexpr (EPI == E_DGELU && r > 0) {
+        if constexpr (EPI == E_DGELU && !AUXF && r > 0) {
           __syncthreads();
           stg_put(img, aux[r & 1], w, lane);
           if constexpr (r < 3) stg_fetch(aux[(r + 1) & 1], tile_rsrc(p.aux, p.ldc, m0, n0), svo, ldc2, r + 1);
@@ -754,7 +823,7 @@
         u16x4 hk[8];
         sfor<0, 16>([&](auto kc) {
           constexpr int kk = decltype(kc)::value, k = 16 * r + kk, i = k >> 3, j = k & 7;
-          if constexpr (EPI == E_DGELU && (kk & 7) == 0) {
+          if constexpr (EPI == E_DGELU && !AUXF && (kk & 7) == 0) {
             sfor<0, 8>([&](auto hc) {
               constexpr int k2 = k + decltype(hc)::value, i2 = k2 >> 3, j2 = k2 & 7;
               hk[decltype(hc)::value] = *reinterpret_cast<const u16x4*>(
@@ -765,12 +834,28 @@
           const uint32_t at = stg_off(32 * wr + 16 * (i & 1) + (lane & 15), lcol + 16 * j);
           u16x4 o;
           if constexpr (EPI == E_DGELU) {
-            const u16x4 hh = hk[kk & 7];
+            u16x4 hh;
+            if constexpr (!AUXF) {
+              hh = hk[kk & 7];
+            } else {
+              const u16x8 hp = r < 2 ? pf[k >> 1] : fa[r & 1][(k >> 1) & 7];
+              hh = (k & 1) ? __builtin_shufflevector(hp, hp, 4, 5, 6, 7) : __builtin_shufflevector(hp, hp, 0, 1, 2, 3);
+            }
 #pragma unroll
             for (int e = 0; e < 4; ++e) {
               const bf16_t gb = f2bf(v[e] * bf2f(hh[e]));
               o[e] = gb;
               cs[j][e] += bf2f(gb);
+            }
+          } else if constexpr (EPI == E_GELU && AUXF) {
+            const gelu_f32x2 u[2] = {{bf2f(f2bf(v[0] + bj[j][0])), bf2f(f2bf(v[1] + bj[j][1]))},
+                                     {bf2f(f2bf(v[2] + bj[j][2])), bf2f(f2bf(v[3] + bj[j][3]))}};
+            gelu_f32x2 y2[2], d2[2];
+            gelu_fwd_grad2n<2>(u, y2, d2);
+#pragma unroll
+            for (int h = 0; h < 2; ++h) {
+              o[2 * h] = f2bf(y2[h][0]); o[2 * h + 1] = f2bf(y2[h][1]);
+              dk[kk][2 * h] = f2bf(d2[h][0]); dk[kk][2 * h + 1] = f2bf(d2[h][1]);
             }
           } else if constexpr (EPI == E_GELU) {
 #pragma unroll
@@ -789,7 +874,14 @@
         __syncthreads();
         stg_read(img, buf, w, lane);
         stg_write_out(buf, rsc, svo, ldc2, r);
-        if constexpr (EPI == E_GELU) {
+        if constexpr (EPI == E_GELU && AUXF) {
+          sfor<0, 8>([&](auto c) {
+            constexpr int q = decltype(c)::value;
+            const u16x8 pr = __builtin_shufflevector(dk[2 * q], dk[2 * q + 1], 0, 1, 2, 3, 4, 5, 6, 7);
+            __builtin_amdgcn_raw_buffer_store_b128(__builtin_bit_cast(u32x4, pr), rsf, (int)fvo, 1024 * (8 * r + q), 0);
+          });
+        }
+        if constexpr (EPI == E_GELU && !AUXF) {
           __syncthreads();
           sfor<0, 16>([&](auto kc) {
             constexpr int kk = decltype(kc)::value, k = 16 * r + kk, i = k >> 3, j = k & 7;
@@ -823,7 +915,7 @@
     if (DIAG) {
       const uint64_t st2 = stamp();
       if (tid == 0) {
-        uint64_t* d = reinterpret_cast<uint64_t*>(p.ws) + 8 * (int64_t)item;
+        uint64_t* d = p.stamps + 8 * (int64_t)item;
         d[0] = st0; d[1] = st1; d[2] = st2; d[3] = rt0;
         for (int i = 0; i < 4; ++i) d[4 + i] = ((uint64_t)ph[2 * i + 1] << 32) | ph[2 * i];
       }
@@ -866,9 +958,19 @@
 }
 
 template <int LAYOUT>
-int launch_asm_layout(int epi, const GemmArgs& a, int splits, hipStream_t s) {
+int launch_asm_layout(int epi, const GemmArgs& a, int splits, bool auxf, hipStream_t s) {
   const int items = (a.M / TM) * (a.N / TN) * splits;
   const dim3 grid(persist_grid(items), 1);
+  if constexpr (LAYOUT == L_NT) {
+    if (auxf && epi == E_GELU) {
+      gemm_asm_kernel<L_NT, E_GELU, 0, false, true><<<grid, NTH, 0, s>>>(a);
+      return (int)hipGetLastError();
+    }
+    if (auxf && epi == E_DGELU) {
+      gemm_asm_kernel<L_NT, E_DGELU, 0, false, true><<<grid, NTH, 0, s>>>(a);
+      return (int)hipGetLastError();
+    }
+  }
   if (use_p3(LAYOUT, a, items, (int)grid.x) && (epi == E_PLAIN || epi == E_BIAS || epi == E_F32)) {
     switch (epi) {
       case E_PLAIN: gemm_asm_kernel<LAYOUT, E_PLAIN, 0, true><<<grid, NTH, 0, s>>>(a); break;
@@ -925,8 +1027,18 @@
 }
 
 template <int LAYOUT>
-int launch_layout(int epi, const GemmArgs& a, int splits, hipStream_t s) {
+int launch_layout(int epi, const GemmArgs& a, int splits, bool auxf, hipStream_t s) {
   const dim3 grid((a.M / TM) * (a.N / TN), splits);
+  if constexpr (LAYOUT == L_NT) {
+    if (auxf && epi == E_GELU) {
+      gemm_kernel<L_NT, E_GELU, true><<<grid, NTH, 0, s>>>(a);
+      return (int)hipGetLastError();
+    }
+    if (auxf && epi == E_DGELU) {
+      gemm_kernel<L_NT, E_DGELU, true><<<grid, NTH, 0, s>>>(a);
+      return (int)hipGetLastError();
+    }
+  }
   switch (epi) {
     case E_PLAIN: gemm_kernel<LAYOUT, E_PLAIN><<<grid, NTH, 0, s>>>(a); break;
     case E_BIAS: gemm_kernel<LAYOUT, E_BIAS><<<grid, NTH, 0, s>>>(a); break;
@@ -955,8 +1067,9 @@
 
 PDT_API int pdt_gemm_bf16(int layout, int epi, const void* A, const void* B, void* C, int64_t M, int64_t N, int64_t K,
                           int64_t lda, int64_t ldb, int64_t ldc, const void* bias, const void* aux, void* aux_out,
-                          void* dbias, float* ws, int splits, hipStream_t s) {
+                          void* dbias, float* ws, int splits, int aux_frag, hipStream_t s) {
   if (!pdt_gemm_ok(layout, M, N, K, lda, ldb, splits) || ldc < N || ldc % 4) return (int)hipErrorInvalidValue;
+  if (aux_frag && (layout != L_NT || (epi != E_GELU && epi != E_DGELU))) return (int)hipErrorInvalidValue;
   if (epi < 0 || epi > E_DGELU) return (int)hipErrorInvalidValue;
   if (splits > 1 && (epi != E_PLAIN || !ws)) return (int)hipErrorInvalidValue;
   if ((epi == E_BIAS || epi == E_GELU) && !bias) return (int)hipErrorInvalidValue;
@@ -971,7 +1084,8 @@
   a.grp = xcd_grp((int)(M / TM), (int)(N / TN), (int)(K / splits), a.xpr);
   const int run_epi = splits > 1 ? E_F32 : epi;
   if (splits > 1) a.ldc = N;
-  int err = layout == L_NT ? launch_layout<L_NT>(run_epi, a, splits, s) : launch_layout<L_TT>(run_epi, a, splits, s);
+  int err = layout == L_NT ? launch_layout<L_NT>(run_epi, a, splits, aux_frag != 0, s)
+                           : launch_layout<L_TT>(run_epi, a, splits, false, s);
   if (err) return err;
   if (splits > 1) {
     const int64_t n4 = M * N / 4;
@@ -985,8 +1099,9 @@
 
 PDT_API int pdt_gemm2_bf16(int layout, int epi, const void* A, const void* B, void* C, int64_t M, int64_t N,
                            int64_t K, int64_t lda, int64_t ldb, int64_t ldc, const void* bias, const void* aux,
-                           void* aux_out, void* dbias, float* ws, int splits, hipStream_t s) {
+                           void* aux_out, void* dbias, float* ws, int splits, int aux_frag, hipStream_t s) {
   if (!pdt_gemm_ok(layout, M, N, K, lda, ldb, splits) || ldc < N || ldc % 8) return (int)hipErrorInvalidValue;
+  if (aux_frag && (layout != L_NT || (epi != E_GELU && epi != E_DGELU))) return (int)hipErrorInvalidValue;
   if (K / splits < 2 * KB) return (int)hipErrorInvalidValue;
   if (epi < 0 || epi > E_DGELU) return (int)hipErrorInvalidValue;
   if (splits > 1 && (epi != E_PLAIN || !ws)) return (int)hipErrorInvalidValue;
@@ -1002,8 +1117,8 @@
   a.grp = xcd_grp((int)(M / TM), (int)(N / TN), (int)(K / splits), a.xpr);
   const int run_epi = splits > 1 ? E_F32 : epi;
   if (splits > 1) a.ldc = N;
-  int err = layout == L_NT ? launch_asm_layout<L_NT>(run_epi, a, splits, s)
-                           : launch_asm_layout<L_TT>(run_epi, a, splits, s);
+  int err = layout == L_NT ? launch_asm_layout<L_NT>(run_epi, a, splits, aux_frag != 0, s)
+                           : launch_asm_layout<L_TT>(run_epi, a, splits, false, s);
   if (err) return err;
   if (splits > 1) {
     if (ldc != N) return (int)hipErrorInvalidValue;
@@ -1024,22 +1139,38 @@
   return pdt_gemm_stamps_epi_bf16(layout, E_PLAIN, A, B, C, M, N, K, lda, ldb, nullptr, nullptr, stamps, s);
 }
 
+PDT_API int pdt_gemm_stamps_aux_bf16(int layout, int epi, const void* A, const void* B, void* C, int64_t M, int64_t N,
+                                     int64_t K, int64_t lda, int64_t ldb, const void* bias, const void* aux,
+                                     void* aux_out, float* ws, int aux_frag, void* stamps, hipStream_t s);
 PDT_API int pdt_gemm_stamps_epi_bf16(int layout, int epi, const void* A, const void* B, void* C, int64_t M, int64_t N,
                                      int64_t K, int64_t lda, int64_t ldb, const void* bias, void* aux_out,
                                      void* stamps, hipStream_t s) {
+  if (epi == E_DGELU) return (int)hipErrorInvalidValue;
+  return pdt_gemm_stamps_aux_bf16(layout, epi, A, B, C, M, N, K, lda, ldb, bias, nullptr, aux_out, nullptr, 0, stamps,
+                                  s);
+}
+
+PDT_API int pdt_gemm_stamps_aux_bf16(int layout, int epi, const void* A, const void* B, void* C, int64_t M, int64_t N,
+                                     int64_t K, int64_t lda, int64_t ldb, const void* bias, const void* aux,
+                                     void* aux_out, float* ws, int aux_frag, void* stamps, hipStream_t s) {
   if (!pdt_gemm_ok(layout, M, N, K, lda, ldb, 1) || K < 2 * KB || !stamps) return (int)hipErrorInvalidValue;
-  if (epi != E_PLAIN && (layout != L_NT || !bias || (epi == E_GELU && !aux_out) || (epi != E_BIAS && epi != E_GELU)))
-    return (int)hipErrorInvalidValue;
+  if (epi < E_PLAIN || epi > E_DGELU || (epi != E_PLAIN && layout != L_NT)) return (int)hipErrorInvalidValue;
+  if ((epi == E_BIAS || epi == E_GELU) && !bias) return (int)hipErrorInvalidValue;
+  if ((epi == E_GELU && !aux_out) || (epi == E_DGELU && (!aux || !ws))) return (int)hipErrorInvalidValue;
+  if (aux_frag && epi != E_GELU && epi != E_DGELU) return (int)hipErrorInvalidValue;
   GemmArgs a{};
-  a.A = (const bf16_t*)A; a.B = (const bf16_t*)B; a.C = C; a.ws = (float*)stamps;
-  a.bias = (const bf16_t*)bias; a.aux_out = (bf16_t*)aux_out;
+  a.A = (const bf16_t*)A; a.B = (const bf16_t*)B; a.C = C; a.ws = ws; a.stamps = (uint64_t*)stamps;
+  a.bias = (const bf16_t*)bias; a.aux = (const bf16_t*)aux; a.aux_out = (bf16_t*)aux_out;
   a.M = (int)M; a.N = (int)N; a.K = (int)K; a.lda = lda; a.ldb = ldb; a.ldc = N; a.k_per_split = (int)K;
   a.xpr = xcd_cut((int)(M / TM), (int)(N / TN));
   a.grp = xcd_grp((int)(M / TM), (int)(N / TN), (int)K, a.xpr);
   const dim3 grid(persist_grid((int)((M / TM) * (N / TN))), 1);
   if (layout == L_TT) gemm_asm_kernel<L_TT, E_PLAIN, 1><<<grid, NTH, 0, s>>>(a);
   else if (epi == E_BIAS) gemm_asm_kernel<L_NT, E_BIAS, 1><<<grid, NTH, 0, s>>>(a);
+  else if (epi == E_GELU && aux_frag) gemm_asm_kernel<L_NT, E_GELU, 1, false, true><<<grid, NTH, 0, s>>>(a);
   else if (epi == E_GELU) gemm_asm_kernel<L_NT, E_GELU, 1><<<grid, NTH, 0, s>>>(a);
+  else if (epi == E_DGELU && aux_frag) gemm_asm_kernel<L_NT, E_DGELU, 1, false, true><<<grid, NTH, 0, s>>>(a);
+  else if (epi == E_DGELU) gemm_asm_kernel<L_NT, E_DGELU, 1><<<grid, NTH, 0, s>>>(a);
   else gemm_asm_kernel<L_NT, E_PLAIN, 1><<<grid, NTH, 0, s>>>(a);
   return (int)hipGetLastError();
 }
diff --git a/pytorch_distributedtraining_amd/ops/gemm.py b/pytorch_distributedtraining_amd/ops/gemm.py
--- a/pytorch_distributedtraining_amd/ops/gemm.py
+++ b/pytorch_distributedtraining_amd/ops/gemm.py
@@ -31,12 +31,25 @@
 KERNEL = {"name": os.environ.get("PDT_GEMM_KERNEL", "asm")}
 
 
-def _launch(layout, epi, a, b, c, m, n, k, bias=None, aux=None, aux_out=None, dbias=None, ws=None, splits=1):
+AUX_LAYOUTS = ("row", "frag")
+AUX_FORCED = os.environ.get("PDT_GELU_AUX", "")
+if AUX_FORCED not in ("",) + AUX_LAYOUTS:
+    raise ValueError(f"PDT_GELU_AUX={AUX_FORCED!r}: expected row or frag")
+
+
+def resolve_aux_layout(requested: str = "row") -> str:
+    if requested not in AUX_LAYOUTS:
+        raise ValueError(f"aux_layout={requested!r}: expected one of {AUX_LAYOUTS}")
+    return AUX_FORCED or requested
+
+
+def _launch(layout, epi, a, b, c, m, n, k, bias=None, aux=None, aux_out=None, dbias=None, ws=None, splits=1,
+            aux_frag=False):
     asm = KERNEL["name"] == "asm" and k // splits >= 128 and c.stride(0) % 8 == 0
     fn = "pdt_gemm2_bf16" if asm else "pdt_gemm_bf16"
     _lib.call(fn, layout, epi, a.data_ptr(), b.data_ptr(), c.data_ptr(), m, n, k, a.stride(0),
               b.stride(0), c.stride(0), _lib.ptr(bias), _lib.ptr(aux), _lib.ptr(aux_out), _lib.ptr(dbias),
-              _lib.ptr(ws), splits, _lib.stream_handle(a.device))
+              _lib.ptr(ws), splits, int(aux_frag), _lib.stream_handle(a.device))
 
 
 def gemm_nt(a: torch.Tensor, b: torch.Tensor, bias: torch.Tensor | None = None) -> torch.Tensor:
@@ -47,22 +60,31 @@
     return c
 
 
-def gemm_nt_gelu(a: torch.Tensor, b: torch.Tensor, bias: torch.Tensor):
+def gemm_nt_gelu(a: torch.Tensor, b: torch.Tensor, bias: torch.Tensor, aux_layout: str = "row"):
     m, k = a.shape
     n = b.shape[0]
     y = torch.empty(m, n, dtype=torch.bfloat16, device=a.device)
     d = torch.empty_like(y)
-    _launch(L_NT, E_GELU, a, b, y, m, n, k, bias=bias, aux_out=d)
+    _launch(L_NT, E_GELU, a, b, y, m, n, k, bias=bias, aux_out=d, aux_frag=_frag(aux_layout))
     return y, d
 
 
-def gemm_nt_dgelu(a: torch.Tensor, b: torch.Tensor, d: torch.Tensor, bias_dtype=torch.bfloat16):
+def _frag(layout: str) -> bool:
+    if layout not in AUX_LAYOUTS:
+        raise ValueError(f"aux_layout={layout!r}: expected one of {AUX_LAYOUTS}")
+    return layout == "frag"
+
+
+def gemm_nt_dgelu(a: torch.Tensor, b: torch.Tensor, d: torch.Tensor, bias_dtype=torch.bfloat16,
+                  aux_layout: str = "row"):
     m, k = a.shape
     n = b.shape[0]
+    assert not _frag(aux_layout) or (d.shape == (m, n) and d.is_contiguous())
     g = torch.empty(m, n, dtype=torch.bfloat16, device=a.device)
     db = torch.empty(n, dtype=torch.bfloat16, device=a.device)
     ws = torch.empty((m // 256 + 64) * n, dtype=torch.float32, device=a.device)
-    _launch(L_NT, E_DGELU, a, b, g, m, n, k, aux=d, dbias=db, ws=ws)
+    _launch(L_NT, E_DGELU, a, b, g, m, n, k, aux=d, dbias=db, ws=ws,
+            aux_frag=_frag(aux_layout))
     return g, db.to(bias_dtype)
 
 
diff --git a/pytorch_distributedtraining_amd/ops/linear.py b/pytorch_distributedtraining_amd/ops/linear.py
--- a/pytorch_distributedtraining_amd/ops/linear.py
+++ b/pytorch_distributedtraining_amd/ops/linear.py
@@ -521,7 +521,8 @@
         from . import gemm as G
         x2 = x.reshape(-1, x.shape[-1])
         x2 = x2 if x2.is_contiguous() and x2.data_ptr() % 16 == 0 else x2.contiguous()
-        y1, d1 = G.gemm_nt_gelu(x2, w1, b1)
+        ctx.aux_layout = G.resolve_aux_layout("frag")
+        y1, d1 = G.gemm_nt_gelu(x2, w1, b1, aux_layout=ctx.aux_layout)
         if r is None:
             out = F.linear(y1, w2, b2)
         else:
@@ -543,7 +544,7 @@
         if ctx.needs_input_grad[4]:
             db2 = take_bias_grad(d2)
             db2 = db2.to(w2.dtype) if db2 is not None else _colsum(d2, w2.dtype)
-        dpre, db1 = G.gemm_nt_dgelu(d2, transpose16(w2), d1, bias_dtype=w1.dtype)
+        dpre, db1 = G.gemm_nt_dgelu(d2, transpose16(w2), d1, bias_dtype=w1.dtype, aux_layout=ctx.aux_layout)
         dw1 = _wgrad_result(w1, dpre, x2) if ctx.needs_input_grad[1] else None
         dx = None
         if ctx.needs_input_grad[0]:
```

Measured after the change: 151,200 tokens/s (median of 2 runs). Within noise of the previous version (+0.0%).
